# spotify-research/llark

Measured on AMD Instinct MI355X. Metric: clips/sec (25 s audio + 128-tok prompt) end-to-end fwd, higher is better.
Workload: dtype fp16x2-split(fp32-class) prior + bf16x2-split(fp32-class) llm; 1 GPU; configs[1]+llm: 8x25s clips -> Jukebox VQ-VAE+36-layer prior -> 240x4800 -> projector -> Llama-2-7B fwd (S=371) logits; clips_per_gpu=8, global_batch=8, audio_samples=1048576, seq_len=371, prior_depth=36, prior_precision=f16x2, prior_layernorm_folded=True, parallelism=dp1 (clip-sharded, no collective), debug_overrides=False

## Files before the change

include/llark_hip.h:

```cpp
#ifndef LLARK_HIP_H
#define LLARK_HIP_H

#include <stdint.h>

#ifdef __cplusplus
extern "C" {
#endif

typedef void* llark_stream_t;

enum {
    LLARK_OK = 0,
    LLARK_ERR_INVALID = -1,
    LLARK_ERR_UNSUPPORTED = -2,
    LLARK_ERR_LAUNCH = -3
};

enum { LLARK_F16 = 0, LLARK_BF16 = 1 };

enum {
    LLARK_EPI_F32 = 0,
    LLARK_EPI_RESID = 1,
    LLARK_EPI_QGELU_SPLIT = 2,
    LLARK_EPI_OUT16 = 3,
    LLARK_EPI_SWIGLU16 = 4,
    LLARK_EPI_SPLIT16 = 5,
    LLARK_EPI_SWIGLU_SPLIT = 6,
    LLARK_EPI_QGELU_SPLIT8 = 7
};

typedef struct llark_workspace* llark_workspace_t;
llark_workspace_t llark_workspace_create(void);
int llark_workspace_destroy(llark_workspace_t ws);

int llark_version(void);
const char* llark_last_error(void);
int llark_device_info(int device, char* arch_name, int arch_name_len);

int llark_resample_sinc_host(const float* x, int64_t n_in, double ratio, const double* win, const double* dwin, int nwin,
                             int num_table, float* y, int64_t n_out);

int llark_flac_info_host(const uint8_t* data, int64_t n, int* sample_rate, int* channels, int* bits_per_sample, int64_t* total_samples);
int llark_flac_decode_host(const uint8_t* data, int64_t n, int32_t* out, int64_t cap_frames, int64_t* decoded_frames, int verify_md5);

int llark_pack_conv_weight(const float* w, float* wp, int cout, int cin, int k, llark_stream_t stream);
int llark_conv1d_f32(const float* x, int n, int cin, int tin, const float* wp, const float* bias, int cout, int k,
                     int stride, int pad, int dil, float* y, int tout, llark_stream_t stream);
int llark_resblock_f32(const float* x, int n, int c, int t, const float* w1p, const float* b1, const float* w2p,
                       const float* b2, int dil, float* y, llark_stream_t stream);
int llark_codebook_norms_f32(const float* k, int bins, int emb, float* kk, llark_stream_t stream);
int llark_codebook_argmin(const float* x, int n, int emb, int t, const float* k, const float* kk, int bins,
                          int64_t* codes, float* min_dist, llark_stream_t stream);
void* llark_vqvae_plan_create(void);
void llark_vqvae_plan_destroy(void* plan);
int llark_vqvae_plan_add_conv(void* plan, const float* wp, const float* bias, int cin, int cout, int k, int stride, int pad);
int llark_vqvae_plan_add_resblock(void* plan, const float* w1p, const float* b1, const float* w2p, const float* b2, int width, int dil);
int llark_vqvae_encode(void* plan, const float* audio, int n, int t, float* buf0, float* buf1, long long buf_elems,
                       const float* codebook, const float* kk, int bins, int64_t* codes, int* t_out, llark_stream_t stream);
int llark_vqvae_stage_f16x2(const float* audio, const void* in_hi, const void* in_lo, int n, int cin, int tin, const float* w0_f32,
                            const void* w0_hi, const void* w0_lo, const float* b0, const void* wr_hi, const void* wr_lo,
                            const float* br, int depth, const int* dil, const void* wo_hi, const void* wo_lo, const float* bo,
                            const int* wexp, void* out_hi, void* out_lo, float* out_f32, llark_stream_t stream);
int llark_vqvae_pack_frag16(const float* w, int cout, int cin, int k, int perm1x1, int exp2, void* hi, void* lo, llark_stream_t stream);

int llark_codebook_argmin_tie(const float* x, int n, int emb, int t, const float* k, const float* kk, int bins, int64_t* codes,
                              float tie_a, float tie_b, int* flag_count, int* flag_list, int cap, llark_stream_t stream);
int llark_vqvae_fix_near_ties(void* plan, const float* audio, int n, int t_samples, int raw_to_tokens, const int* flag_list, int count,
                              int halo_tokens, int win_tokens, float* win, int* col, float* buf0, float* buf1, long long buf_elems,
                              const float* codebook, const float* kk, int bins, int64_t* codes, llark_stream_t stream);

int llark_prior_embed(const int64_t* z, int n, int t, int width, int bins, const float* x_emb, const float* pos_emb,
                      const float* x_cond, const float* y_cond, float* h, llark_stream_t stream);
int llark_layernorm_split_f16(const float* x, int ldx, int rows, int width, const float* gamma, const float* beta,
                              float eps, void* out_hi, void* out_lo, int ldo, llark_stream_t stream);
int llark_prior_attn(const float* qkv, int ldq, int n, int t, int n_state, int heads, int blocks, int pattern,
                     void* out_hi, void* out_lo, int ldo, llark_stream_t stream);
int llark_layernorm_split_lo8(const float* x, int ldx, int rows, int width, const float* gamma, const float* beta,
                              float eps, void* out_hi, int ldo, void* out_lo8, int ldo8, int sa, llark_stream_t stream);
int llark_prior_attn_lo8(const float* qkv, int ldq, int n, int t, int n_state, int heads, int blocks, int pattern,
                         void* out_hi, int ldo, void* out_lo8, int ldo8, int sa, llark_stream_t stream);
int llark_pool_window(const float* h, int n, int t, int width, int frame_len, float* out, int frames,
                      llark_stream_t stream);
int llark_pool_mean(const float* h, int n, int t, int width, const int* lens, float* out, llark_stream_t stream);
int llark_zero_pad16(void* plane, int rows, int ld, int from, llark_stream_t stream);

int llark_gemm16(int dtype, int split, int epilogue, const void* a_hi, const void* a_lo, int lda, const void* wt,
                 int ldw, const float* bias, int m, int n, int kp, float* c, int ldc, const float* resid, int ldr,
                 void* out_hi, void* out_lo, int ldo, llark_stream_t stream);
int llark_gemm16_ex(int variant, int dtype, int split, int epilogue, const void* a_hi, const void* a_lo, int lda,
                    const void* wt, int ldw, const float* bias, int m, int n, int kp, float* c, int ldc, const float* resid,
                    int ldr, void* out_hi, void* out_lo, int ldo, llark_stream_t stream);
int llark_gemm16_ws(int variant, int dtype, int split, int epilogue, const void* a_hi, const void* a_lo, int lda,
                    const void* wt, int ldw, const float* bias, int m, int n, int kp, float* c, int ldc, const float* resid,
                    int ldr, void* out_hi, void* out_lo, int ldo, llark_workspace_t ws, llark_stream_t stream);

int llark_gemm16_ln_takes(int m, int n, int kp);
int llark_gemm16_ln(int dtype, int epilogue, const void* a_hi, const void* a_lo, int lda, const void* wt, int ldw, const float* bias, int m,
                    int n, int kp, float* c, int ldc, const float* resid, int ldr, void* out_hi, void* out_lo, int ldo,
                    const float* ln_stat, const float* ln_vec, float* ln_part, llark_workspace_t ws, llark_stream_t stream);
int llark_ln_stats_finalize(const float* part, int rows, int nparts, int width, float eps, float* stat, llark_stream_t stream);
int llark_gemm16_ln_p(int dtype, int epilogue, const void* a_hi, const void* a_lo, int lda, const void* wt, int ldw, const float* bias, int m,
                      int n, int kp, float* c, int ldc, const float* resid, int ldr, void* out_hi, void* out_lo, int ldo,
                      const float* ln_stat, const float* ln_vec, float* ln_part, const float* ln_pred, llark_workspace_t ws, llark_stream_t stream);
int llark_ln_stats_finalize_p(const float* part, int rows, int nparts, int width, float eps, float* stat, float* pred, llark_stream_t stream);
int llark_gemm16_lnp_fragw(int dtype, const void* a_hi, const void* a_lo, int lda, const void* wfrag, const float* bias, int m, int n, int kp,
                           float* c, int ldc, const float* resid, int ldr, void* out_hi, void* out_lo, int ldo, const float* ln_vec,
                           float* ln_part, const float* ln_pred, llark_stream_t stream);
int llark_ln_row_pred(const float* x, int ldx, int rows, int width, float eps, float* pred, llark_stream_t stream);
int llark_gemm16_lo8(int epilogue, const void* a_hi, const void* a_lo8, int lda, int lda8, const void* wt, int ldw,
                     const void* w8, int ldw8, const float* bias, int m, int n, int kp, int sa, int sw, float* c, int ldc, const float* resid, int ldr,
                     void* out_hi, void* out_lo8, int ldo, int ldo8, llark_workspace_t ws, llark_stream_t stream);
int llark_pack_weight_lo8(const void* wt, int ldw, int n, int kp, int sw, void* out, int ldo, llark_stream_t stream);
int llark_pack_weight16_frag(const void* wt, int ldw, int n, int kp, void* dst, llark_stream_t stream);
int llark_gemm16_fragw(int variant, int dtype, int split, int epilogue, const void* a_hi, const void* a_lo, int lda,
                       const void* wfrag, const float* bias, int m, int n, int kp, float* c, int ldc, const float* resid,
                       int ldr, void* out_hi, void* out_lo, int ldo, llark_stream_t stream);
int llark_gemm16_fragw_whole_tiles(int split, int epilogue, int m, int n, int kp);
int llark_gemm16_fragw_rope_qkv(const void* a_hi, const void* a_lo, int lda, const void* wfrag, int kp, int batch, int s, int nh, int hd,
                                int pos0, const float* cos_t, const float* sin_t, int max_pos, void* q, void* k_cache, void* vt_cache,
                                void* q_lo, void* k_cache_lo, void* vt_cache_lo, int smax, llark_stream_t stream);
long long llark_gemm16_sk_scratch_bytes(void);
int llark_gemm16_fragw_sk(int variant, int dtype, int split, int epilogue, const void* a_hi, const void* a_lo, int lda,
                          const void* wfrag, const float* bias, int m, int n, int kp, float* c, int ldc, const float* resid,
                          int ldr, void* out_hi, void* out_lo, int ldo, void* scratch, long long scratch_bytes,
                          llark_stream_t stream);
int llark_gemm16_resid_rmsnorm(int dtype, int split, const void* a_hi, const void* a_lo, int lda, const void* wt, int ldw,
                               int m, int n, int kp, float* h, int ldh, const float* norm_w, float eps, void* x_hi,
                               void* x_lo, int ldx, llark_stream_t stream);
int llark_gemm16_rmsnorm_a(int dtype, int split, int epilogue, const float* x, int ldx, const float* norm_w, float eps,
                           const void* wt, int ldw, const float* bias, int m, int n, int kp, float* c, int ldc, void* out_hi,
                           void* out_lo, int ldo, llark_stream_t stream);
int llark_gemm16_batched(int dtype, int split, int epilogue, const void* a_hi, const void* a_lo, int lda, long long stride_a,
                         const void* wt, int ldw, long long stride_w, int m, int n, int kp, float* c, int ldc,
                         long long stride_c, void* out_hi, void* out_lo, int ldo, long long stride_o, int batch,
                         llark_stream_t stream);
int llark_pack_weight16(const void* w, int src_dtype, int transpose, int k, int n, void* wt, int dst_dtype, int ldw,
                        llark_stream_t stream);
int llark_split16(int dtype, const float* x, int ldx, int rows, int width, void* out_hi, void* out_lo, int ldo,
                  llark_stream_t stream);


int llark_embed_gather(const int64_t* ids, int rows, const void* table, int table_dtype, int vocab, int width,
                       float* out, int ldo, llark_stream_t stream);
int llark_rmsnorm_bf16(const float* x, int ldx, int rows, int width, const float* w, float eps, void* out_hi,
                       void* out_lo, int ldo, llark_stream_t stream);
int llark_rope_split_heads(const float* qkv, int batch, int s, int nh, int hd, int pos0, const float* cos_t,
                           const float* sin_t, int max_pos, void* q, void* k_cache, void* vt_cache, void* q_lo,
                           void* k_cache_lo, void* vt_cache_lo, int smax, llark_stream_t stream);
int llark_attn_prefill_bf16(const void* q, const void* k_cache, const void* vt_cache, const void* q_lo,
                            const void* k_cache_lo, const void* vt_cache_lo, int batch, int s, int nh, int hd, int past,
                            int smax, void* out, void* out_lo, llark_stream_t stream);
int llark_attn_decode_bf16(const void* q, const void* k_cache, const void* vt_cache, const void* q_lo,
                           const void* k_cache_lo, const void* vt_cache_lo, int batch, int nh, int hd, int total, int smax,
                           void* out, void* out_lo, llark_stream_t stream);
int llark_attn_prefill_bf16_alibi(const void* q, const void* k_cache, const void* vt_cache, const void* q_lo,
                                  const void* k_cache_lo, const void* vt_cache_lo, int batch, int s, int nh, int hd, int past,
                                  int smax, void* out, void* out_lo, const float* alibi_slopes, llark_stream_t stream);
int llark_attn_decode_bf16_alibi(const void* q, const void* k_cache, const void* vt_cache, const void* q_lo,
                                 const void* k_cache_lo, const void* vt_cache_lo, int batch, int nh, int hd, int total, int smax,
                                 void* out, void* out_lo, const float* alibi_slopes, llark_stream_t stream);

int llark_gemv16_dma(int split, int epilogue, const void* a_hi, const void* a_lo, int lda, const void* wt, int ldw, const float* bias,
                     int m, int n, int kp, float* c, int ldc, const float* resid, int ldr, void* out_hi, void* out_lo, int ldo,
                     llark_stream_t stream);
int llark_gemv16_dma_rmsnorm(int split, int epilogue, const float* x, int ldx, const float* norm_w, float eps, const void* wt, int ldw,
                             const float* bias, int m, int n, int kp, float* c, int ldc, void* out_hi, void* out_lo, int ldo,
                             llark_stream_t stream);

int llark_gemm16_t(int dtype, int epilogue, int trans_a, int trans_b, const void* a, int lda, const void* wt, int ldw, int m, int n,
                   int kp, float* c, int ldc, const float* resid, int ldr, llark_stream_t stream);
int llark_gemm16_t_sumsq(int dtype, int epilogue, int trans_a, int trans_b, const void* a, int lda, const void* wt, int ldw, int m, int n,
                         int kp, float* c, int ldc, const float* resid, int ldr, double* sumsq, llark_stream_t stream);

int llark_gemm16_t_ex(int variant, int dtype, int epilogue, int trans_a, int trans_b, const void* a, int lda, const void* wt, int ldw, int m,
                      int n, int kp, float* c, int ldc, const float* resid, int ldr, double* sumsq, llark_stream_t stream);

int llark_attn_prefill_bf16_lse(const void* q, const void* k_cache, const void* vt_cache, int batch, int s, int nh, int hd,
                                int smax, void* out, float* lse, const float* alibi_slopes, llark_stream_t stream);
int llark_attn_backward_bf16(const void* q, const void* k_cache, const void* v_rm, const void* dO, const void* o, const float* lse,
                             float* dsum, int batch, int s, int nh, int hd, int smax, float* dq, float* dk, float* dv,
                             const float* alibi_slopes, llark_stream_t stream);

int llark_layernorm_bf16(const float* x, int ldx, int rows, int width, const float* gamma, const float* beta, float eps,
                         void* out_hi, void* out_lo, int ldo, llark_stream_t stream);
int llark_layernorm_f32(const float* x, int ldx, int rows, int width, const float* gamma, const float* beta, float eps,
                        float* y, int ldy, llark_stream_t stream);
int llark_clamp_f32(float* x, long long n, float limit, llark_stream_t stream);
int llark_clamp_bwd_bf16(const float* x, long long n, float limit, void* dy, llark_stream_t stream);
int llark_scale_f32(float* x, long long n, float a, llark_stream_t stream);
int llark_gelu_split_bf16(const float* x, int ldx, int rows, int width, void* out_hi, void* out_lo, int ldo,
                          llark_stream_t stream);
int llark_layernorm_bwd(const float* x, int ldx, const float* gamma, const float* dy, int ldy, int rows, int width, float eps,
                        float* dx, int lddx, float* dgamma, float* dbeta, int accumulate, llark_stream_t stream);
int llark_gelu_bwd(const float* up, const float* dact, long long n, float* dup32, void* dup16, llark_stream_t stream);
int llark_causal_softmax_rows_alibi(const float* scores, int batch, int s, float scale, const float* slopes, int nh, void* p_out,
                                    int ldp, llark_stream_t stream);
int llark_clap_logmel(const float* wav, int batch, int n, int quantize_int16, const float* window, const float* twiddle,
                      const float* melw, const int* mel_lo, const int* mel_hi, float* out, llark_stream_t stream);
int llark_clap_patchify(const float* x, int batch, int frames, int mel, const float* bn_mean, const float* bn_scale,
                        const float* bn_bias, const int* tap_idx, const float* tap_w, int spec, int patch, void* out_hi,
                        void* out_lo, int ldo, llark_stream_t stream);
int llark_clap_window_attn(const float* qkv, int ldq, int batch, int H, int W, int C, int heads, int window, int shift,
                           const float* bias_table, void* out_hi, void* out_lo, void* out_hi_dup, int ldo, llark_stream_t stream);
int llark_layernorm_bf16_dup(const float* x, int ldx, int rows, int width, const float* gamma, const float* beta, float eps,
                             void* out_hi, void* out_lo, void* out_hi_dup, int ldo, llark_stream_t stream);
int llark_gemm16_act(int variant, int dtype, int split, int epilogue, const void* a_hi, const void* a_lo, int lda, const void* wt,
                     int ldw, const float* bias, int m, int n, int kp, void* out_hi, void* out_lo, void* out_hi_dup, int ldo,
                     int act, llark_stream_t stream);
int llark_clap_patch_merge(const float* x, int ldx, int batch, int H, int W, int C, float* out, int ldo, llark_stream_t stream);
int llark_mean_rows_f32(const float* x, int ldx, int batch, int L, int C, float* out, int ldo, llark_stream_t stream);
int llark_relu_split_bf16(const float* x, int ldx, int rows, int width, void* out_hi, void* out_lo, int ldo, llark_stream_t stream);
int llark_l2_normalize_rows(float* x, int ldx, int rows, int width, float eps, llark_stream_t stream);

int llark_attn_decode_rope_bf16(const float* qkv, int batch, int nh, int hd, int pos, const int* pos_dev, const float* cos_t,
                                const float* sin_t, int max_pos, void* k_cache, void* vt_cache, void* k_cache_lo, void* vt_cache_lo,
                                int smax, void* out, void* out_lo, const float* alibi_slopes, llark_stream_t stream);
#define LLARK_ROW_IDLE 0
#define LLARK_ROW_ACTIVE 1
#define LLARK_ROW_FINISHED 2
int llark_attn_decode_rope_bf16_rows(const float* qkv, int batch, int nh, int hd, const int* pos_rows, const float* cos_t,
                                     const float* sin_t, int max_pos, void* k_cache, void* vt_cache, void* k_cache_lo, void* vt_cache_lo,
                                     int smax, void* out, void* out_lo, const float* alibi_slopes, llark_stream_t stream);
int llark_decode_advance_rows(const float* logits, int ldl, int vocab, int batch, const int64_t* choice, int* pos_rows, int* state,
                              int64_t* next_ids, int64_t* out_col, int ld_out, int64_t eos, int64_t pad, llark_stream_t stream);
int llark_rope_split_heads_dpos(const float* qkv, int batch, int nh, int hd, const int* pos_dev, const float* cos_t,
                                const float* sin_t, void* q, void* k_cache, void* vt_cache, void* q_lo, void* k_cache_lo,
                                void* vt_cache_lo, int smax, llark_stream_t stream);
int llark_attn_decode_bf16_dpos(const void* q, const void* k_cache, const void* vt_cache, const void* q_lo,
                                const void* k_cache_lo, const void* vt_cache_lo, int batch, int nh, int hd,
// ... 62 lines not shown
```

llark_amd/_lib.py:

```python
from __future__ import annotations

import ctypes
import os
import subprocess
from ctypes import c_char_p, c_double, c_float, c_int, c_int64, c_uint, c_void_p

_HERE = os.path.dirname(os.path.abspath(__file__))
LIB_PATH = os.environ.get("LLARK_HIP_LIB") or os.path.join(_HERE, "libllark_hip.so")
CSRC = os.path.join(_HERE, "csrc")

_lib = None


class LlarkHipError(RuntimeError):
    pass


def build(force: bool = False, verbose: bool = False) -> str:
    srcs = [os.path.join(CSRC, f) for f in os.listdir(CSRC) if f.endswith((".hip", ".h"))]
    srcs.append(os.path.join(_HERE, "..", "include", "llark_hip.h"))
    stale = (not os.path.exists(LIB_PATH)) or any(
        os.path.getmtime(s) > os.path.getmtime(LIB_PATH) for s in srcs if os.path.exists(s)
    )
    if force or stale:
        cmd = ["make", "-C", CSRC, "-j8"] + (["-B"] if force else [])
        res = subprocess.run(cmd, capture_output=not verbose, text=True)
        if res.returncode != 0:
            raise LlarkHipError(f"building libllark_hip.so failed:\n{res.stdout}\n{res.stderr}")
    return LIB_PATH


_P = c_void_p
_SIGS = {
    "llark_version": [],
    "llark_device_info": [c_int, c_char_p, c_int],
    "llark_resample_sinc_host": [_P, c_int64, c_double, _P, _P, c_int, c_int, _P, c_int64],
    "llark_flac_info_host": [_P, c_int64, _P, _P, _P, _P],
    "llark_flac_decode_host": [_P, c_int64, _P, c_int64, _P, c_int],
    "llark_pack_conv_weight": [_P, _P, c_int, c_int, c_int, _P],
    "llark_conv1d_f32": [_P, c_int, c_int, c_int, _P, _P, c_int, c_int, c_int, c_int, c_int, _P, c_int, _P],
    "llark_resblock_f32": [_P, c_int, c_int, c_int, _P, _P, _P, _P, c_int, _P, _P],
    "llark_codebook_norms_f32": [_P, c_int, c_int, _P, _P],
    "llark_codebook_argmin": [_P, c_int, c_int, c_int, _P, _P, c_int, _P, _P, _P],
    "llark_prior_embed": [_P, c_int, c_int, c_int, c_int, _P, _P, _P, _P, _P, _P],
    "llark_layernorm_split_f16": [_P, c_int, c_int, c_int, _P, _P, c_float, _P, _P, c_int, _P],
    "llark_prior_attn": [_P, c_int, c_int, c_int, c_int, c_int, c_int, c_int, _P, _P, c_int, _P],
    "llark_pool_window": [_P, c_int, c_int, c_int, c_int, _P, c_int, _P],
    "llark_pool_mean": [_P, c_int, c_int, c_int, _P, _P, _P],
    "llark_zero_pad16": [_P, c_int, c_int, c_int, _P],
    "llark_vqvae_plan_add_conv": [_P, _P, _P, c_int, c_int, c_int, c_int, c_int],
    "llark_vqvae_plan_add_resblock": [_P, _P, _P, _P, _P, c_int, c_int],
    "llark_vqvae_encode": [_P, _P, c_int, c_int, _P, _P, c_int64, _P, _P, c_int, _P, _P, _P],
    "llark_codebook_argmin_tie": [_P, c_int, c_int, c_int, _P, _P, c_int, _P, c_float, c_float, _P, _P, c_int, _P],
    "llark_vqvae_fix_near_ties": [_P, _P, c_int, c_int, c_int, _P, c_int, c_int, c_int, _P, _P, _P, _P, c_int64, _P, _P, c_int, _P, _P],
    "llark_vqvae_stage_f16x2": [_P, _P, _P, c_int, c_int, c_int, _P, _P, _P, _P, _P, _P, _P, c_int, _P, _P, _P, _P, _P, _P, _P, _P, _P],
    "llark_vqvae_pack_frag16": [_P, c_int, c_int, c_int, c_int, c_int, _P, _P, _P],
    "llark_gemm16": [c_int, c_int, c_int, _P, _P, c_int, _P, c_int, _P, c_int, c_int, c_int, _P, c_int, _P, c_int,
                     _P, _P, c_int, _P],
    "llark_gemm16_ex": [c_int, c_int, c_int, c_int, _P, _P, c_int, _P, c_int, _P, c_int, c_int, c_int, _P, c_int, _P, c_int,
                        _P, _P, c_int, _P],
    "llark_gemm16_ws": [c_int, c_int, c_int, c_int, _P, _P, c_int, _P, c_int, _P, c_int, c_int, c_int, _P, c_int, _P, c_int,
                        _P, _P, c_int, _P, _P],
    "llark_gemm16_lo8": [c_int, _P, _P, c_int, c_int, _P, c_int, _P, c_int, _P, c_int, c_int, c_int, c_int, c_int, _P, c_int, _P, c_int,
                         _P, _P, c_int, c_int, _P, _P],
    "llark_pack_weight_lo8": [_P, c_int, c_int, c_int, c_int, _P, c_int, _P],
    "llark_gemm16_ln_takes": [c_int, c_int, c_int],
    "llark_gemm16_ln": [c_int, c_int, _P, _P, c_int, _P, c_int, _P, c_int, c_int, c_int, _P, c_int, _P, c_int, _P, _P, c_int, _P, _P, _P, _P, _P],
    "llark_ln_stats_finalize": [_P, c_int, c_int, c_int, c_float, _P, _P],
    "llark_gemm16_fragw_whole_tiles": [c_int, c_int, c_int, c_int, c_int],
    "llark_gemm16_ln_p": [c_int, c_int, _P, _P, c_int, _P, c_int, _P, c_int, c_int, c_int, _P, c_int, _P, c_int, _P, _P, c_int, _P, _P, _P, _P, _P, _P],
    "llark_gemm16_lnp_fragw": [c_int, _P, _P, c_int, _P, _P, c_int, c_int, c_int, _P, c_int, _P, c_int, _P, _P, c_int, _P, _P, _P, _P],
    "llark_ln_stats_finalize_p": [_P, c_int, c_int, c_int, c_float, _P, _P, _P],
    "llark_ln_row_pred": [_P, c_int, c_int, c_int, c_float, _P, _P],
    "llark_workspace_destroy": [_P],
    "llark_layernorm_split_lo8": [_P, c_int, c_int, c_int, _P, _P, c_float, _P, c_int, _P, c_int, c_int, _P],
    "llark_prior_attn_lo8": [_P, c_int, c_int, c_int, c_int, c_int, c_int, c_int, _P, c_int, _P, c_int, c_int, _P],
    "llark_pack_weight16_frag": [_P, c_int, c_int, c_int, _P, _P],
    "llark_gemm16_fragw": [c_int, c_int, c_int, c_int, _P, _P, c_int, _P, _P, c_int, c_int, c_int, _P, c_int, _P, c_int,
                           _P, _P, c_int, _P],
    "llark_gemm16_fragw_sk": [c_int, c_int, c_int, c_int, _P, _P, c_int, _P, _P, c_int, c_int, c_int, _P, c_int, _P, c_int,
                              _P, _P, c_int, _P, c_int64, _P],
    "llark_gemm16_fragw_rope_qkv": [_P, _P, c_int, _P, c_int, c_int, c_int, c_int, c_int, c_int, _P, _P, c_int, _P, _P, _P, _P, _P, _P, c_int, _P],
    "llark_gemm16_resid_rmsnorm": [c_int, c_int, _P, _P, c_int, _P, c_int, c_int, c_int, c_int, _P, c_int, _P, c_float, _P, _P,
                                   c_int, _P],
    "llark_gemm16_rmsnorm_a": [c_int, c_int, c_int, _P, c_int, _P, c_float, _P, c_int, _P, c_int, c_int, c_int, _P, c_int, _P, _P,
                               c_int, _P],
    "llark_gemm16_batched": [c_int, c_int, c_int, _P, _P, c_int, c_int64, _P, c_int, c_int64, c_int, c_int, c_int, _P, c_int,
                             c_int64, _P, _P, c_int, c_int64, c_int, _P],
    "llark_pack_weight16": [_P, c_int, c_int, c_int, c_int, _P, c_int, c_int, _P],
    "llark_split16": [c_int, _P, c_int, c_int, c_int, _P, _P, c_int, _P],
    "llark_embed_gather": [_P, c_int, _P, c_int, c_int, c_int, _P, c_int, _P],
    "llark_rmsnorm_bf16": [_P, c_int, c_int, c_int, _P, c_float, _P, _P, c_int, _P],
    "llark_attn_prefill_bf16_alibi": [_P, _P, _P, _P, _P, _P, c_int, c_int, c_int, c_int, c_int, c_int, _P, _P, _P, _P],
    "llark_attn_decode_bf16_alibi": [_P, _P, _P, _P, _P, _P, c_int, c_int, c_int, c_int, c_int, _P, _P, _P, _P],
    "llark_gemv16_dma": [c_int, c_int, _P, _P, c_int, _P, c_int, _P, c_int, c_int, c_int, _P, c_int, _P, c_int, _P, _P, c_int, _P],
    "llark_gemv16_dma_rmsnorm": [c_int, c_int, _P, c_int, _P, c_float, _P, c_int, _P, c_int, c_int, c_int, _P, c_int, _P, _P, c_int, _P],
    "llark_gemm16_t": [c_int, c_int, c_int, c_int, _P, c_int, _P, c_int, c_int, c_int, c_int, _P, c_int, _P, c_int, _P],
    "llark_gemm16_t_ex": [c_int, c_int, c_int, c_int, c_int, _P, c_int, _P, c_int, c_int, c_int, c_int, _P, c_int, _P, c_int, _P, _P],
    "llark_gemm16_t_sumsq": [c_int, c_int, c_int, c_int, _P, c_int, _P, c_int, c_int, c_int, c_int, _P, c_int, _P, c_int, _P, _P],
    "llark_attn_prefill_bf16_lse": [_P, _P, _P, c_int, c_int, c_int, c_int, c_int, _P, _P, _P, _P],
    "llark_attn_backward_bf16": [_P, _P, _P, _P, _P, _P, _P, c_int, c_int, c_int, c_int, c_int, _P, _P, _P, _P, _P],
    "llark_layernorm_bf16": [_P, c_int, c_int, c_int, _P, _P, c_float, _P, _P, c_int, _P],
    "llark_layernorm_f32": [_P, c_int, c_int, c_int, _P, _P, c_float, _P, c_int, _P],
    "llark_clamp_f32": [_P, c_int64, c_float, _P],
    "llark_clamp_bwd_bf16": [_P, c_int64, c_float, _P, _P],
    "llark_sumsq_f32": [_P, c_int64, _P, c_int, _P],
    "llark_scale_f32": [_P, c_int64, c_float, _P],
    "llark_gelu_split_bf16": [_P, c_int, c_int, c_int, _P, _P, c_int, _P],
    "llark_layernorm_bwd": [_P, c_int, _P, _P, c_int, c_int, c_int, c_float, _P, c_int, _P, _P, c_int, _P],
    "llark_gelu_bwd": [_P, _P, c_int64, _P, _P, _P],
    "llark_causal_softmax_rows_alibi": [_P, c_int, c_int, c_float, _P, c_int, _P, c_int, _P],
    "llark_clap_logmel": [_P, c_int, c_int, c_int, _P, _P, _P, _P, _P, _P, _P],
    "llark_clap_patchify": [_P, c_int, c_int, c_int, _P, _P, _P, _P, _P, c_int, c_int, _P, _P, c_int, _P],
    "llark_clap_window_attn": [_P, c_int, c_int, c_int, c_int, c_int, c_int, c_int, c_int, _P, _P, _P, _P, c_int, _P],
    "llark_layernorm_bf16_dup": [_P, c_int, c_int, c_int, _P, _P, c_float, _P, _P, _P, c_int, _P],
    "llark_gemm16_act": [c_int, c_int, c_int, c_int, _P, _P, c_int, _P, c_int, _P, c_int, c_int, c_int, _P, _P, _P, c_int, c_int, _P],
    "llark_clap_patch_merge": [_P, c_int, c_int, c_int, c_int, c_int, _P, c_int, _P],
    "llark_mean_rows_f32": [_P, c_int, c_int, c_int, c_int, _P, c_int, _P],
    "llark_relu_split_bf16": [_P, c_int, c_int, c_int, _P, _P, c_int, _P],
    "llark_l2_normalize_rows": [_P, c_int, c_int, c_int, c_float, _P],
    "llark_attn_decode_rope_bf16": [_P, c_int, c_int, c_int, c_int, _P, _P, _P, c_int, _P, _P, _P, _P, c_int, _P, _P, _P, _P],
    "llark_attn_decode_rope_bf16_rows": [_P, c_int, c_int, c_int, _P, _P, _P, c_int, _P, _P, _P, _P, c_int, _P, _P, _P, _P],
    "llark_decode_advance_rows": [_P, c_int, c_int, c_int, _P, _P, _P, _P, _P, c_int, c_int64, c_int64, _P],
    "llark_rope_split_heads_dpos": [_P, c_int, c_int, c_int, _P, _P, _P, _P, _P, _P, _P, _P, _P, c_int, _P],
    "llark_attn_decode_bf16_dpos": [_P, _P, _P, _P, _P, _P, c_int, c_int, c_int, _P, c_int, _P, _P, _P],
    "llark_rope_split_heads": [_P, c_int, c_int, c_int, c_int, c_int, _P, _P, c_int, _P, _P, _P, _P, _P, _P, c_int, _P],
    "llark_attn_prefill_bf16": [_P, _P, _P, _P, _P, _P, c_int, c_int, c_int, c_int, c_int, c_int, _P, _P, _P],
    "llark_attn_decode_bf16": [_P, _P, _P, _P, _P, _P, c_int, c_int, c_int, c_int, c_int, _P, _P, _P],
    "llark_cross_entropy_shifted": [_P, c_int, c_int, c_int, c_int, _P, c_int64, _P, _P, _P],
    "llark_transpose16": [_P, c_int, c_int, c_int, _P, c_int, c_int, c_int64, c_int64, _P],
    "llark_split_heads16": [_P, c_int, c_int, c_int, c_int, _P, _P],
    "llark_causal_softmax_rows": [_P, c_int, c_int, c_float, _P, c_int, _P],
    "llark_attn_ds": [_P, _P, c_int, c_int, c_float, _P, c_int, _P],
    "llark_rope_merge_bwd": [_P, _P, _P, _P, _P, c_int, c_int, c_int, c_int, c_int, _P, _P],
    "llark_rmsnorm_bwd": [_P, _P, _P, c_int, c_int, c_float, _P, c_int, _P, _P],
    "llark_rmsnorm_bwd_out16": [_P, _P, _P, c_int, c_int, c_float, _P, c_int, _P, _P, c_int, _P],
    "llark_swiglu_fwd": [_P, c_int, c_int, _P, _P],
    "llark_swiglu_bwd": [_P, _P, c_int, c_int, _P, _P],
    "llark_cross_entropy_bwd": [_P, c_int, c_int, c_int, c_int, _P, _P, _P, c_float, _P, c_int, _P],
    "llark_colsum_f32": [_P, c_int, c_int, c_int, _P, _P],
    "llark_gather_rows_f32": [_P, c_int, _P, c_int, c_int, _P, c_int, _P],
    "llark_scatter_add_rows_f32": [_P, c_int, _P, c_int, c_int, _P, c_int, _P],
    "llark_adamw": [c_int, _P, _P, _P, _P, c_int64, c_float, c_float, c_float, c_float, c_float, c_int, c_float, _P],
    "llark_adamw_clip": [c_int, _P, _P, _P, _P, c_int64, c_float, c_float, c_float, c_float, c_float, c_int, c_float, _P, c_float, _P],
    "llark_gemm16_fragw_swiglu_train": [c_int, _P, c_int, _P, c_int, c_int, c_int, _P, c_int, _P, c_int, _P],
    "llark_pack_frag_t16": [_P, c_int, c_int, c_int, _P, _P],
    "llark_gemm16_ta_fragw": [c_int, _P, c_int, _P, c_int, c_int, c_int, _P, c_int, _P, c_int, _P, _P],
    "llark_pack_frag_t16x16": [_P, c_int, c_int, c_int, _P, _P],
    "llark_gemm16_ta_fragw16": [c_int, _P, c_int, _P, c_int, c_int, c_int, _P, c_int, _P, c_int, _P, _P],
    "llark_gemm16_fragw_rope_qkv_train": [_P, c_int, _P, c_int, c_int, c_int, c_int, c_int, c_int, _P, _P, c_int, _P, _P, _P, c_int, _P, _P],
    "llark_attn_backward_bf16_fused": [_P, _P, _P, _P, c_int, _P, _P, _P, c_int, c_int, c_int, c_int, c_int, _P, _P, c_int, c_int, _P, _P],
    "llark_gemv16_dma_blocks": [c_int, c_int],
    "llark_gemv16_dma_chain": [c_int, c_int, _P, _P, c_int, _P, c_int, _P, c_float, _P, c_int, _P, c_int, c_int, c_int, _P, c_int, _P, c_int, _P, _P, c_int, _P, c_uint, _P, _P],
    "llark_attn_decode_rope_bf16_chain": [_P, c_int, c_int, c_int, c_int, _P, _P, _P, c_int, _P, _P, _P, _P, c_int, _P, _P, _P, _P, _P],
    "llark_adamw_twins": [_P, _P, _P, _P, c_int, c_int, c_float, c_float, c_float, c_float, c_float, c_int, c_float, _P, c_float, _P, c_int, _P, _P],
}


def declared_symbols():
    return sorted(list(_SIGS.keys()) + ["llark_last_error", "llark_vqvae_plan_create", "llark_vqvae_plan_destroy", "llark_workspace_create", "llark_gemm16_sk_scratch_bytes"])


_recorder = None
current_label = None


class _RecordingProxy:
    def __init__(self, real, rec):
        self._real, self._rec = real, rec

    def __getattr__(self, name):
        fn = getattr(self._real, name)
        if not name.startswith("llark_") or name == "llark_last_error":
            return fn
        rec = self._rec

        def call(*args):
            rc = fn(*args)
            rec.append((fn, name, args, current_label))
            return rc

        return call


def set_recorder(rec) -> None:
    global _recorder
    _recorder = rec


def lib():
    L = _real_lib()
    return _RecordingProxy(L, _recorder) if _recorder is not None else L


def _real_lib():
    global _lib
    if _lib is None:
        if not os.path.exists(LIB_PATH):
            build()
# ... 27 lines not shown
```

llark_amd/csrc/gemm.hip:

```cpp

#ifndef GEMM_ABLATE
#define GEMM_ABLATE 0
#endif

#include <new>

#include "gemm_core.h"
#include "gemm_rope_epi.h"
#include "gemm_bd.h"
#include "gemm_bda_loop.h"

namespace llark {

template <typename T, bool SPLIT, int EPI, typename C>
__device__ __forceinline__ void gemm_tile(const GemmParams& p, int bid, char* smem) {
    typedef typename Mfma<T>::frag frag;
    constexpr int STAGE = (SPLIT ? 2 : 1) * C::A_BYTES + C::B_BYTES;
    constexpr int OFF_L = C::A_BYTES, OFF_W = (SPLIT ? 2 : 1) * C::A_BYTES;
    constexpr int NS = C::NSTAGE;

    const int lane = threadIdx.x & 63;
    const int w = __builtin_amdgcn_readfirstlane(threadIdx.x >> 6);
    const int wm = w / C::WN, wn = w % C::WN;

// ... 647 lines not shown
        case 1: return dispatch<T, Cfg1>(p, split, epi, s);
        case 2: return dispatch<T, Cfg2>(p, split, epi, s);
        case 11: return dispatch<T, Cfg11>(p, split, epi, s);
        case 12: return dispatch<T, Cfg12>(p, split, epi, s);
        case 13:
            if (split) break;
            switch (epi) {
                case EPI_F32: return launch_gemm<T, false, EPI_F32, Cfg13>(p, s);
                case EPI_RESID: return launch_gemm<T, false, EPI_RESID, Cfg13>(p, s);
                case EPI_OUT16: return launch_gemm<T, false, EPI_OUT16, Cfg13>(p, s);
                case EPI_SWIGLU16: return launch_gemm<T, false, EPI_SWIGLU16, Cfg13>(p, s);
            }
            break;
        case 32: {
            if (split && ws && ws->cus % 8 == 0) {
                GemmParams q = p;
                const int dt = std::is_same<T, half_t>::value ? LLARK_F16 : LLARK_BF16;
                if (ws_begin(ws, q, s) == 0) {
                    const int rc = launch_gemm256x(q, dt, epi, s, ws->cus);
                    if (rc != -1000) {
                        ws_end(ws, cdiv(p.M, 256) * cdiv(p.N, 256), ws->cus / 8);
                        return rc;
                    }
                }
            }
        }
        [[fallthrough]];
        case 31: {
            if (split && ws && ws->cus % 8 == 0) {
                GemmParams q = p;
                const int dt = std::is_same<T, half_t>::value ? LLARK_F16 : LLARK_BF16;
                if (ws_begin(ws, q, s) == 0) {
                    const int rc = launch_gemm256n(q, dt, epi, s, ws->cus);
                    if (rc != -1000) {
                        ws_end(ws, cdiv(p.M, 256) * cdiv(p.N, 256), ws->cus / 8);
                        return rc;
                    }
                }
            }
        }
        [[fallthrough]];
        case 30: {
            if (split && ws && ws->cus % 8 == 0) {
                GemmParams q = p;
                const int dt = std::is_same<T, half_t>::value ? LLARK_F16 : LLARK_BF16;
                if (ws_begin(ws, q, s) == 0) {
                    const int rc = launch_gemm256(q, dt, epi, s, ws->cus);
                    if (rc != -1000) {
                        ws_end(ws, cdiv(p.M, 256) * cdiv(p.N, 256), ws->cus / 8);
                        return rc;
                    }
                }
            }
        }
        [[fallthrough]];
        case 20: {
            const int rc = dispatch_persist<T, Cfg12>(p, split, epi, s, ws);
            return rc == -1000 ? dispatch<T, Cfg12>(p, split, epi, s) : rc;
        }
    }
    set_error("gemm: unknown tile variant %d", variant);
    return LLARK_ERR_INVALID;
}

}

using namespace llark;

static int pick_variant(int split, int m, int n, int kp, bool has_ws) {
    if (m <= 128) return 0;
    if (!split && kp % 64 == 0 && n < 16384) return 11;
    if (n < 256) return 0;
    if (kp % 64 != 0) return kp < 2048 ? 1 : 2;
    const bool persist = has_ws;
    if (split && persist && kp >= 128 && (long)cdiv(m, 256) * cdiv(n, 256) >= 384) return kp >= 2048 ? 32 : 31;
    if (kp < 2048) return 12;
    if (m >= 16384 && persist) return 20;
    if (!split && n < 16384) return 11;
    return 12;
}

static int gemm16_impl(int variant, int dtype, int split, int epilogue, const void* a_hi, const void* a_lo, int lda,
                       const void* wt, int ldw, const float* bias, int m, int n, int kp, float* c, int ldc,
                       const float* resid, int ldr, void* out_hi, void* out_lo, int ldo, int batch, long long sa,
                       long long sw, long long sc, long long sr, long long so, llark_stream_t stream, void* out_hi2 = nullptr,
                       int act = 0, llark_workspace* ws = nullptr) {
    LLARK_REQUIRE(a_hi && wt && m > 0 && n > 0 && kp > 0, "gemm16: null pointer or empty problem");
    LLARK_REQUIRE(kp % 64 == 0 || (kp % 32 == 0 && variant < 10),
                  "gemm16: kp=%d must be a multiple of the K-step (zero-pad K)", kp);
    LLARK_REQUIRE(lda % 8 == 0 && ldw % 8 == 0 && lda >= kp && ldw >= kp, "gemm16: lda/ldw must be >= kp and multiples of 8");
    LLARK_REQUIRE(!split || a_lo, "gemm16: split mode needs the lo plane");
    LLARK_REQUIRE(((uintptr_t)a_hi & 15) == 0 && ((uintptr_t)wt & 15) == 0 && (!a_lo || ((uintptr_t)a_lo & 15) == 0),
                  "gemm16: operands must be 16-byte aligned");
    if (epilogue == EPI_F32 || epilogue == EPI_RESID) LLARK_REQUIRE(c && ldc >= n, "gemm16: fp32 output missing");
    if (epilogue == EPI_RESID) LLARK_REQUIRE(resid && ldr >= n, "gemm16: residual missing");
    if (epilogue == EPI_QGELU_SPLIT || epilogue == EPI_SPLIT16) LLARK_REQUIRE(out_hi && out_lo && ldo >= n, "gemm16: split outputs missing");
    if (epilogue == EPI_OUT16) LLARK_REQUIRE(out_hi && ldo >= n, "gemm16: 16-bit output missing");
    if (IS_SWIGLU(epilogue)) LLARK_REQUIRE(out_hi && n % 64 == 0 && ldo >= n / 2, "gemm16: swiglu needs n%%64==0 and an output");
    if (epilogue == EPI_SWIGLU_SPLIT) LLARK_REQUIRE(out_lo, "gemm16: swiglu-split needs the lo output");
    GemmParams p = {};
    p.Ahi = a_hi; p.Alo = a_lo; p.lda = lda; p.Wt = wt; p.ldw = ldw; p.bias = bias;
    p.M = m; p.N = n; p.Kp = kp; p.C = c; p.ldc = ldc; p.R = resid; p.ldr = ldr;
    p.Ohi = out_hi; p.Olo = out_lo; p.ldo = ldo; p.Ohi2 = out_hi2; p.act = act;
    p.tiles_m = p.tiles_n = 0;
    p.batch = batch; p.sA = sa; p.sW = sw; p.sC = sc; p.sR = sr; p.sO = so;
    hipStream_t s = (hipStream_t)stream;
    if (variant < 0 && m <= 16 && batch <= 1 && act == 0 && !out_hi2) {
        int rc = 1;
        if (dtype == LLARK_F16) rc = dispatch_skinny<half_t>(p, split != 0, epilogue, s);
        else if (dtype == LLARK_BF16) rc = dispatch_skinny<bf16_t>(p, split != 0, epilogue, s);
        if (rc != 1) return rc;
    }
    if (variant < 0) variant = pick_variant(split, m, n, kp, ws != nullptr);
    if (dtype == LLARK_F16) return dispatch_variant<half_t>(variant, p, split != 0, epilogue, s, ws);
    if (dtype == LLARK_BF16) return dispatch_variant<bf16_t>(variant, p, split != 0, epilogue, s, ws);
    set_error("gemm16: unknown dtype %d", dtype);
    return LLARK_ERR_INVALID;
}

extern "C" int llark_gemm16_ex(int variant, int dtype, int split, int epilogue, const void* a_hi, const void* a_lo, int lda,
                               const void* wt, int ldw, const float* bias, int m, int n, int kp, float* c, int ldc,
                               const float* resid, int ldr, void* out_hi, void* out_lo, int ldo,
                               llark_stream_t stream) {
    return gemm16_impl(variant, dtype, split, epilogue, a_hi, a_lo, lda, wt, ldw, bias, m, n, kp, c, ldc, resid, ldr, out_hi,
                       out_lo, ldo, 0, 0, 0, 0, 0, 0, stream);
}

extern "C" int llark_gemm16_ws(int variant, int dtype, int split, int epilogue, const void* a_hi, const void* a_lo, int lda,
                               const void* wt, int ldw, const float* bias, int m, int n, int kp, float* c, int ldc,
                               const float* resid, int ldr, void* out_hi, void* out_lo, int ldo, llark_workspace_t ws,
                               llark_stream_t stream) {
    return gemm16_impl(variant, dtype, split, epilogue, a_hi, a_lo, lda, wt, ldw, bias, m, n, kp, c, ldc, resid, ldr, out_hi,
                       out_lo, ldo, 0, 0, 0, 0, 0, 0, stream, nullptr, 0, ws);
}

extern "C" int llark_gemm16_ln_takes(int m, int n, int kp) { return gemm256x_takes(m, n, kp) ? 1 : 0; }

extern "C" int llark_gemm16_ln(int dtype, int epilogue, const void* a_hi, const void* a_lo, int lda, const void* wt, int ldw, const float* bias, int m,
                               int n, int kp, float* c, int ldc, const float* resid, int ldr, void* out_hi, void* out_lo, int ldo,
                               const float* ln_stat, const float* ln_vec, float* ln_part, llark_workspace_t ws, llark_stream_t stream) {
    return llark_gemm16_ln_p(dtype, epilogue, a_hi, a_lo, lda, wt, ldw, bias, m, n, kp, c, ldc, resid, ldr, out_hi, out_lo, ldo, ln_stat, ln_vec, ln_part,
                             nullptr, ws, stream);
}

extern "C" int llark_gemm16_ln_p(int dtype, int epilogue, const void* a_hi, const void* a_lo, int lda, const void* wt, int ldw, const float* bias, int m,
                                 int n, int kp, float* c, int ldc, const float* resid, int ldr, void* out_hi, void* out_lo, int ldo,
                                 const float* ln_stat, const float* ln_vec, float* ln_part, const float* ln_pred, llark_workspace_t ws,
                                 llark_stream_t stream) {
    LLARK_REQUIRE(a_hi && a_lo && wt && ln_vec && ws && m > 0 && n > 0 && kp > 0, "gemm16_ln: null pointer or empty problem");
    LLARK_REQUIRE(ln_pred == nullptr || ln_part != nullptr, "gemm16_ln: ln_pred belongs to the producer role (ln_part)");
    LLARK_REQUIRE((ln_stat != nullptr) != (ln_part != nullptr), "gemm16_ln: exactly one of ln_stat (consumer) / ln_part (producer) must be given");
    LLARK_REQUIRE(lda % 8 == 0 && ldw % 8 == 0 && lda >= kp && ldw >= kp, "gemm16_ln: lda/ldw must be >= kp and multiples of 8");
    if (ln_part) LLARK_REQUIRE(epilogue == EPI_RESID && c && resid && out_hi && out_lo && ldc >= n && ldr >= n && ldo >= n, "gemm16_ln: the producer role is LLARK_EPI_RESID with c, resid and the operand planes");
    else LLARK_REQUIRE((epilogue == EPI_F32 && c && ldc >= n) || (epilogue == EPI_QGELU_SPLIT && out_hi && out_lo && ldo >= n), "gemm16_ln: the consumer role is LLARK_EPI_F32 or LLARK_EPI_QGELU_SPLIT");
    if (!gemm256x_takes(m, n, kp) || ws->cus % 8) {
        set_error("gemm16_ln: m=%d n=%d kp=%d is not a shape the 256x256 tile takes", m, n, kp);
        return LLARK_ERR_UNSUPPORTED;
    }
    GemmParams p = {};
    p.Ahi = a_hi; p.Alo = a_lo; p.lda = lda; p.Wt = wt; p.ldw = ldw; p.bias = bias;
    p.M = m; p.N = n; p.Kp = kp; p.C = c; p.ldc = ldc; p.R = resid; p.ldr = ldr;
    p.Ohi = out_hi; p.Olo = out_lo; p.ldo = ldo;
    p.ln_stat = ln_stat; p.ln_vec = ln_vec; p.ln_part = ln_part; p.ln_pred = ln_pred;
    hipStream_t s = (hipStream_t)stream;
    if (ws_begin(ws, p, s)) {
        set_error("gemm16_ln: workspace without counters");
        return LLARK_ERR_INVALID;
    }
    const int rc = launch_gemm256x(p, dtype, epilogue, s, ws->cus);
    if (rc == -1000) {
        set_error("gemm16_ln: operands do not meet the tile's alignment rules");
        return LLARK_ERR_UNSUPPORTED;
    }
    ws_end(ws, cdiv(m, 256) * cdiv(n, 256), ws->cus / 8);
    return rc;
}

extern "C" int llark_gemm16_lnp_fragw(int dtype, const void* a_hi, const void* a_lo, int lda, const void* wfrag, const float* bias, int m, int n, int kp,
                                      float* c, int ldc, const float* resid, int ldr, void* out_hi, void* out_lo, int ldo, const float* ln_vec,
                                      float* ln_part, const float* ln_pred, llark_stream_t stream) {
    LLARK_REQUIRE(a_hi && a_lo && wfrag && ln_vec && ln_part && c && resid && out_hi && out_lo && m > 0 && n > 0 && kp > 0,
                  "gemm16_lnp_fragw: null pointer or empty problem");
    LLARK_REQUIRE(kp % 64 == 0 && lda % 8 == 0 && lda >= kp && ldc >= n && ldr >= n && ldo >= n, "gemm16_lnp_fragw: kp must be a multiple of 64, lda >= kp a multiple of 8, ldc / ldr / ldo >= n");
    LLARK_REQUIRE(((uintptr_t)a_hi & 15) == 0 && ((uintptr_t)a_lo & 15) == 0 && ((uintptr_t)wfrag & 15) == 0, "gemm16_lnp_fragw: operands must be 16-byte aligned");
    GemmParams p = {};
    p.Ahi = a_hi; p.Alo = a_lo; p.lda = lda; p.Wt = wfrag; p.ldw = 0; p.bias = bias; p.M = m; p.N = n; p.Kp = kp;
    p.C = c; p.ldc = ldc; p.R = resid; p.ldr = ldr; p.Ohi = out_hi; p.Olo = out_lo; p.ldo = ldo;
    p.ln_vec = ln_vec; p.ln_part = ln_part; p.ln_pred = ln_pred;
    const int rc = launch_gemm_bda_lnp(p, dtype, (hipStream_t)stream);
    if (rc == -1000) {
        set_error("gemm16_lnp_fragw: needs f16 / bf16 planes, kp >= 192, n %% 4 == 0, 16-byte aligned fp32 rows (ldc, ldr multiples of 4) and 8-byte aligned plane rows (ldo a multiple of 4)");
        return LLARK_ERR_UNSUPPORTED;
    }
    return rc;
}

extern "C" llark_workspace_t llark_workspace_create(void) {
    int dev = 0, cus = 0;
    if (hipGetDevice(&dev) != hipSuccess || hipDeviceGetAttribute(&cus, hipDeviceAttributeMultiprocessorCount, dev) != hipSuccess) {
        set_error("workspace_create: cannot query the current device");
        return nullptr;
    }
    llark_workspace* ws = new (std::nothrow) llark_workspace();
    if (!ws) { set_error("workspace_create: out of host memory"); return nullptr; }
    ws->device = dev; ws->cus = cus; ws->base = 0; ws->counters = nullptr;
#ifdef G256X_PROF
    if (const char* e = getenv("LLARK_G256X_CUS")) ws->cus = atoi(e);
#endif
    if (hipMalloc((void**)&ws->counters, LLARK_WS_BYTES) != hipSuccess || hipMemset(ws->counters, 0, LLARK_WS_BYTES) != hipSuccess) {
        set_error("workspace_create: cannot allocate %d bytes of device memory", LLARK_WS_BYTES);
        if (ws->counters) (void)hipFree(ws->counters);
        delete ws;
        return nullptr;
    }
    return ws;
}

extern "C" int llark_workspace_destroy(llark_workspace_t ws) {
    if (!ws) return LLARK_OK;
    if (ws->counters) (void)hipFree(ws->counters);
    delete ws;
    return LLARK_OK;
}

extern "C" int llark_gemm16_lo8(int epilogue, const void* a_hi, const void* a_lo8, int lda, int lda8, const void* wt, int ldw,
                                const void* w8, int ldw8, const float* bias, int m, int n, int kp, int sa, int sw, float* c, int ldc, const float* resid,
                                int ldr, void* out_hi, void* out_lo8, int ldo, int ldo8, llark_workspace_t ws,
                                llark_stream_t stream) {
    LLARK_REQUIRE(a_hi && a_lo8 && wt && w8 && ws && m > 0 && n > 0, "gemm16_lo8: null pointer (a_hi / a_lo8 / wt / w8 / ws) or empty problem");
    LLARK_REQUIRE(kp % 64 == 0 && kp >= 128, "gemm16_lo8: kp=%d must be a multiple of 64 and >= 128 (zero-pad K)", kp);
    LLARK_REQUIRE(lda % 8 == 0 && ldw % 8 == 0 && lda >= kp && ldw >= kp && lda8 >= kp && lda8 % 16 == 0,
                  "gemm16_lo8: lda/ldw/lda8 must be >= kp, lda/ldw multiples of 8, lda8 a multiple of 16");
    LLARK_REQUIRE(((uintptr_t)a_hi & 15) == 0 && ((uintptr_t)wt & 15) == 0 && ((uintptr_t)a_lo8 & 15) == 0,
                  "gemm16_lo8: operands must be 16-byte aligned");
    LLARK_REQUIRE(sa >= 0 && sa <= 40 && sw >= -40 && sw <= 40, "gemm16_lo8: scale exponents out of range (sa=%d sw=%d)", sa, sw);
    LLARK_REQUIRE(ldw8 >= kp && ldw8 % 16 == 0 && ((uintptr_t)w8 & 15) == 0, "gemm16_lo8: w8 plane needs ldw8 >= kp, ldw8 %% 16 == 0 and 16-byte alignment");
    if (epilogue == EPI_F32 || epilogue == EPI_RESID) LLARK_REQUIRE(c && ldc >= n, "gemm16_lo8: fp32 output missing");
    if (epilogue == EPI_RESID) LLARK_REQUIRE(resid && ldr >= n, "gemm16_lo8: residual missing");
    if (epilogue == EPI_QGELU_SPLIT8)
        LLARK_REQUIRE(out_hi && out_lo8 && ldo >= n && ldo8 >= ((n + 63) & ~63) && ldo8 % 64 == 0,
                      "gemm16_lo8: split outputs missing (ldo8 must cover n rounded up to 64 and be a multiple of 64)");
    LLARK_REQUIRE(epilogue == EPI_F32 || epilogue == EPI_RESID || epilogue == EPI_QGELU_SPLIT8, "gemm16_lo8: unsupported epilogue %d", epilogue);
    LLARK_REQUIRE(ws->cus > 0 && ws->cus % 8 == 0, "gemm16_lo8: device with %d CUs is not supported (needs a multiple of 8)", ws->cus);
    GemmParams p = {};
    p.Ahi = a_hi; p.Alo = a_lo8; p.lda = lda; p.lda8 = lda8; p.Wt = wt; p.ldw = ldw; p.bias = bias;
    p.M = m; p.N = n; p.Kp = kp; p.C = c; p.ldc = ldc; p.R = resid; p.ldr = ldr;
    p.Ohi = out_hi; p.Olo = out_lo8; p.ldo = ldo; p.ldo8 = ldo8; p.lo8_sa = sa; p.lo8_sw = sw; p.W8 = w8; p.ldw8 = ldw8;
    hipStream_t s = (hipStream_t)stream;
    if (ws_begin(ws, p, s)) { set_error("gemm16_lo8: workspace unusable"); return LLARK_ERR_LAUNCH; }
    const int rc = launch_gemm256_lo8n(p, epilogue, s, ws->cus);
    if (rc == -1000) { set_error("gemm16_lo8: problem outside the kernel's range (32-bit operand offsets)"); return LLARK_ERR_UNSUPPORTED; }
    ws_end(ws, cdiv(m, 256) * cdiv(n, 256), ws->cus / 8);
    return rc;
}

extern "C" int llark_gemm16_act(int variant, int dtype, int split, int epilogue, const void* a_hi, const void* a_lo, int lda,
                                const void* wt, int ldw, const float* bias, int m, int n, int kp, void* out_hi, void* out_lo,
                                void* out_hi_dup, int ldo, int act, llark_stream_t stream) {
    LLARK_REQUIRE(epilogue == EPI_SPLIT16 || epilogue == EPI_OUT16, "gemm16_act: epilogue must be SPLIT16 or OUT16");
    LLARK_REQUIRE(act == 0 || act == 2, "gemm16_act: act must be 0 (none) or 2 (exact GELU)");
    LLARK_REQUIRE(!out_hi_dup || epilogue == EPI_SPLIT16, "gemm16_act: the duplicate hi plane belongs to the SPLIT16 epilogue");
    return gemm16_impl(variant, dtype, split, epilogue, a_hi, a_lo, lda, wt, ldw, bias, m, n, kp, nullptr, 0, nullptr, 0, out_hi,
                       out_lo, ldo, 0, 0, 0, 0, 0, 0, stream, out_hi_dup, act);
}

extern "C" int llark_pack_weight16_frag(const void* wt, int ldw, int n, int kp, void* dst, llark_stream_t stream) {
    LLARK_REQUIRE(wt && dst && n > 0 && kp > 0 && kp % 64 == 0 && ldw >= kp && ldw % 8 == 0, "pack_weight16_frag: bad arguments (kp must be a multiple of 64)");
    LLARK_REQUIRE(((uintptr_t)wt & 15) == 0 && ((uintptr_t)dst & 15) == 0, "pack_weight16_frag: pointers must be 16-byte aligned");
    const long long total = (long long)cdiv(n, 32) * (kp / 16) * 64;
    pack_frag_kernel<<<dim3((unsigned)((total + 255) / 256)), 256, 0, (hipStream_t)stream>>>((const unsigned short*)wt, ldw, n, kp, (uint4*)dst, total);
    return check_launch("pack_weight16_frag");
}

static int llark_device_cus() {
    static int cached[64] = {0};
    int dev = 0;
    if (hipGetDevice(&dev) != hipSuccess || dev < 0 || dev >= 64) return 256;
    if (!cached[dev]) {
        int cus = 0;
        if (hipDeviceGetAttribute(&cus, hipDeviceAttributeMultiprocessorCount, dev) != hipSuccess || cus <= 0) return 256;
        cached[dev] = cus;
    }
    return cached[dev];
}

static bool fragw_sk_rule(bool split, int m, int n, int kp) {
    const long long tiles_bd0 = (long long)cdiv(m, CfgBD0::BM) * cdiv(n, CfgBD0::BN);
    return (split && tiles_bd0 < 2LL * llark_device_cus()) ||
           (!split && (4 * tiles_bd0 <= 2LL * llark_device_cus() || (tiles_bd0 < 2LL * llark_device_cus() && kp >= 8192)));
}
static bool fragw_small_tiles(int dtype, bool split, int epilogue, int n) {
    if (GEMM_BDA >= 2 && dtype == LLARK_BF16) return false;
    return !split && !IS_SWIGLU(epilogue) && n <= 4096;
}

extern "C" int llark_gemm16_fragw_whole_tiles(int split, int epilogue, int m, int n, int kp) {
    if (m <= 0 || n <= 0 || kp <= 0) return 0;
    return (!fragw_sk_rule(split != 0, m, n, kp) && !fragw_small_tiles(LLARK_BF16, split != 0, epilogue, n)) ? 1 : 0;
}

static int gemm16_fragw_impl(int variant, int dtype, int split, int epilogue, const void* a_hi, const void* a_lo, int lda,
                             const void* wfrag, const float* bias, int m, int n, int kp, float* c, int ldc,
                             const float* resid, int ldr, void* out_hi, void* out_lo, int ldo, void* scratch, long long scratch_bytes,
                             llark_stream_t stream) {
    LLARK_REQUIRE(a_hi && wfrag && m > 0 && n > 0 && kp > 0 && kp % 64 == 0, "gemm16_fragw: null pointer / empty problem / kp not a multiple of 64");
    LLARK_REQUIRE(lda % 8 == 0 && lda >= kp, "gemm16_fragw: lda must be >= kp and a multiple of 8");
    LLARK_REQUIRE(!split || a_lo, "gemm16_fragw: split mode needs the lo plane");
// ... 167 lines not shown
```

llark_amd/csrc/gemm256x.hip:

```cpp
#include "gemm_core.h"

namespace llark {

struct Cfg256X {
    static constexpr int BK = 64, BM = 256, BN = 256, NW = 8, THREADS = 512, MINW = 2;
    static constexpr int TM = 4, TN = 8;
    static constexpr int ROWB = 128, UNIT = 128 * ROWB;
    static constexpr int NW_SLOTS = 3, NA_SLOTS = 7;
    static constexpr int O_W = 0, O_A = NW_SLOTS * UNIT;
    static constexpr int LDS = O_A + NA_SLOTS * UNIT;
    static_assert(LDS == 160 * 1024, "LDS map");
};

template <typename T>
struct Mfma16;
template <>
struct Mfma16<half_t> {
    typedef half8_t frag;
    typedef half4_t out4;
    static __device__ __forceinline__ f32x4_t run(frag a, frag b, f32x4_t c) { return __builtin_amdgcn_mfma_f32_16x16x32_f16(a, b, c, 0, 0, 0); }
};
template <>
struct Mfma16<bf16_t> {
    typedef bf16x8_t frag;
// ... 373 lines not shown
                                if constexpr (i >= r0 + 10 && i < r0 + 14) al[i - r0 - 10][1] = *(const frag*)(smem + vAs[1] + 8192 + (i - r0 - 10) * 2048);
                                if constexpr (i == 16) bf[0] = *(const frag*)(smem + vWs[1]);
                                if constexpr (i == 17) bf[1] = *(const frag*)(smem + vWs[1] + 2048);
                                if constexpr (i >= 18 && i < 22) dmaop(std::integral_constant<int, i - 18>{});
                            } else {
                                if constexpr (i == r0) bf[2] = *(const frag*)(smem + vWs[0] + 2 * 2048);
                                if constexpr (i == r0 + 1) bf[3] = *(const frag*)(smem + vWs[0] + 3 * 2048);
                                if constexpr (i >= r0 + 2 && i < r0 + 6) dmaop(std::integral_constant<int, i - r0 - 2>{});
                                if constexpr (i == 16) bf[0] = *(const frag*)(smem + vWs[1]);
                                if constexpr (i == 17) bf[1] = *(const frag*)(smem + vWs[1] + 2048);
                            }
                        } else {
                            if constexpr (i == 2) bf[2] = *(const frag*)(smem + vWs[1] + 2 * 2048);
                            if constexpr (i == 3) bf[3] = *(const frag*)(smem + vWs[1] + 3 * 2048);
                            if constexpr (i >= 4 && i < 6) midop(std::integral_constant<int, i - 4>{});
                        }
                        __builtin_amdgcn_sched_barrier(0);
                    });
                });
            };

            auto kstep = [&](auto right_tag, int k, int aq, int wL) __attribute__((always_inline)) {
                const int kn = k + 1 < nk ? k + 1 : nk - 1;
                const int wR = wL + 1 >= 3 ? wL - 2 : wL + 1, wN = wL + 2 >= 3 ? wL - 1 : wL + 2;
                const int an = wrap7(aq + 4);
                const int amine = wrap7(aq + wm) * C::UNIT;
                auto reqQ = [&](int j, int lo_plane, int slot) __attribute__((always_inline)) {
                    const unsigned vo = j == 0 ? voA[0] : j == 1 ? voA[1] : j == 2 ? voA[2] : voA[3];
                    dma(lo_plane ? rAl : rAh, vo, kn << 7, C::O_A + slot * C::UNIT + wb + (lo_plane ? 8192 : 0));
                };
                auto reqW = [&](int right, int piece, int slot) __attribute__((always_inline)) {
                    dma(rW, voW[2 * right + piece], kn << 7, C::O_W + slot * C::UNIT + piece * 8192 + wb);
                };
                phase(std::integral_constant<int, 0>{}, std::integral_constant<int, 4>{}, std::true_type{}, amine, wL * C::UNIT,
                      [&](auto ic) __attribute__((always_inline)) { constexpr int i = decltype(ic)::value; reqQ(i >> 1, i & 1, wrap7(an + (i >> 1))); },
                      [&](auto ic) __attribute__((always_inline)) { reqW(0, decltype(ic)::value, wN); });
                __builtin_amdgcn_s_barrier();
                phase(std::integral_constant<int, 1>{}, std::integral_constant<int, 4>{}, right_tag, amine, wR * C::UNIT,
                      [&](auto ic) __attribute__((always_inline)) { constexpr int i = decltype(ic)::value; reqQ(2 + (i >> 1), i & 1, wrap7(an + 2 + (i >> 1))); },
                      [&](auto ic) __attribute__((always_inline)) { reqW(1, decltype(ic)::value, wL); });
                VMCNT(2);
                __builtin_amdgcn_s_barrier();
            };

#if G256X_PRIO
            if (w >= 4) __builtin_amdgcn_s_setprio(1);
#endif
            if (w >= 4) __builtin_amdgcn_s_barrier();
            {
                int aq = 0, wL = 0;
                if (n0 + 128 < p.N) {
                    for (int k = 0; k < nk; ++k) {
                        kstep(std::true_type{}, k, aq, wL);
                        aq = wrap7(aq + 4);
                        wL = wL + 2 >= 3 ? wL - 1 : wL + 2;
                    }
                } else {
                    for (int k = 0; k < nk; ++k) {
                        kstep(std::false_type{}, k, aq, wL);
                        aq = wrap7(aq + 4);
                        wL = wL + 2 >= 3 ? wL - 1 : wL + 2;
                    }
                }
            }
            if (w < 4) __builtin_amdgcn_s_barrier();
            VMCNT(0);
            __builtin_amdgcn_s_barrier();
            PROF_STAMP(1);
            f32x4_t bias[C::TN], res0[C::TN], res1[C::TN];
            f32x4_t gv;
            float2 st[C::TM];
            if (LN != 0) gv = gamma_load(p, n0, wn, lane);
            else epilogue_load_bias(p, bias, n0, wn, lane);
            if (LN == 1 || LN == 2) {
                const bool whole = m0 + C::BM <= p.M;
                const float* rowst = LN == 1 ? p.ln_stat : p.ln_pred;
#pragma unroll
                for (int tm = 0; tm < C::TM; ++tm) {
                    const int m = m0 + wm * 64 + tm * 16 + (lane & 15);
                    st[tm] = (rowst != nullptr && (whole || m < p.M)) ? *(const float2*)(rowst + 2 * (size_t)m) : make_float2(0.f, 1.f);
                }
            }
            epilogue_load_resid<EPI>(p, res0, 0, m0, n0, wm, wn, lane);
            epilogue_load_resid<EPI>(p, res1, 1, m0, n0, wm, wn, lane);
            if (LN != 0) gamma_park(smem, gv, w, lane);
            __builtin_amdgcn_sched_barrier(0);
            if (ch + 1 < nchunks) {
                if (threadIdx.x == 0) __hip_atomic_fetch_add(cnt, 1, __ATOMIC_RELAXED, __HIP_MEMORY_SCOPE_AGENT);
                arrived = true;
                const int nl = (ch + 1) * p.slots + slot_id;
                primed = nl < bandn;
                if (primed) {
                    int m1, n1;
                    tile_of(band0 + nl, m1, n1);
                    set_offsets(m1, n1);
                    prologue();
                }
            }
            __builtin_amdgcn_sched_barrier(0);
            epilogue_store<T, EPI, LN>(p, smem, acc, res0, bias, st, 0, m0, n0, wm, wn, lane);
            __builtin_amdgcn_sched_barrier(0);
            epilogue_load_resid<EPI>(p, res0, 2, m0, n0, wm, wn, lane);
            __builtin_amdgcn_sched_barrier(0);
            epilogue_store<T, EPI, LN>(p, smem, acc, res1, bias, st, 1, m0, n0, wm, wn, lane);
            __builtin_amdgcn_sched_barrier(0);
            epilogue_load_resid<EPI>(p, res1, 3, m0, n0, wm, wn, lane);
            __builtin_amdgcn_sched_barrier(0);
            epilogue_store<T, EPI, LN>(p, smem, acc, res0, bias, st, 2, m0, n0, wm, wn, lane);
            epilogue_store<T, EPI, LN>(p, smem, acc, res1, bias, st, 3, m0, n0, wm, wn, lane);
            PROF_STAMP(2);
            ++prof_tile;
        }
        if (ch + 1 < nchunks) {
            if (threadIdx.x == 0) {
                if (!arrived) __hip_atomic_fetch_add(cnt, 1, __ATOMIC_RELAXED, __HIP_MEMORY_SCOPE_AGENT);
                const int target = p.sync_base + (ch + 1 - G256X_RUNAHEAD) * p.slots;
                for (int it = 0; it < 100000 && __hip_atomic_load(cnt, __ATOMIC_RELAXED, __HIP_MEMORY_SCOPE_AGENT) - target < 0; ++it)
                    __builtin_amdgcn_s_sleep(8);
            }
            __builtin_amdgcn_s_barrier();
        }
    }
#ifdef G256X_PROF
    VMCNT(0);
    __builtin_amdgcn_s_barrier();
    PROF_STAMP(0);
#endif
}

template <typename T, int EPI, int LN>
static int launch256x(GemmParams p, hipStream_t s, int cus) {
    typedef Cfg256X C;
    auto kern = gemm256x_kernel<T, EPI, LN>;
    static PerDeviceOnce once;
    if (once.first()) {
        if (hipFuncSetAttribute((const void*)kern, hipFuncAttributeMaxDynamicSharedMemorySize, C::LDS) != hipSuccess) return -1000;
    }
    p.tiles_m = cdiv(p.M, C::BM);
    p.tiles_n = cdiv(p.N, C::BN);
#ifdef G256X_PROF
    if (const char* e = getenv("LLARK_G256X_PROF_BUF")) p.prof = (long long*)strtoull(e, nullptr, 0);
#endif
    p.slots = cus / 8;
    kern<<<dim3(cus), C::THREADS, C::LDS, s>>>(p);
    return check_launch("gemm256x");
}

template <typename T>
static int dispatch256x(const GemmParams& p, int epi, hipStream_t s, int cus) {
    if (p.ln_stat) {
        if (!p.ln_vec || p.ln_part) return -1000;
        if (epi == EPI_F32) return launch256x<T, EPI_F32, 1>(p, s, cus);
        if (epi == EPI_QGELU_SPLIT) return launch256x<T, EPI_QGELU_SPLIT, 1>(p, s, cus);
        return -1000;
    }
    if (p.ln_part) {
        if (!p.ln_vec || epi != EPI_RESID || !p.Ohi || !p.Olo) return -1000;
        return launch256x<T, EPI_RESID, 2>(p, s, cus);
    }
    switch (epi) {
        case EPI_F32: return launch256x<T, EPI_F32, 0>(p, s, cus);
        case EPI_RESID: return launch256x<T, EPI_RESID, 0>(p, s, cus);
        case EPI_QGELU_SPLIT: return launch256x<T, EPI_QGELU_SPLIT, 0>(p, s, cus);
        case EPI_SPLIT16: if (p.act == 0 && p.Ohi2 == nullptr) return launch256x<T, EPI_SPLIT16, 0>(p, s, cus);
    }
    return -1000;
}

bool gemm256x_takes(int m, int n, int kp) {
    return kp % 64 == 0 && kp >= 128 && n % 4 == 0 && m > 0 && (long)cdiv(m, 256) * cdiv(n, 256) >= 384;
}

int launch_gemm256x(const GemmParams& p, int dtype, int epi, hipStream_t s, int cus) {
    if (!p.Alo || p.Kp % 64 != 0 || p.Kp < 128 || p.batch > 1 || !p.sync || cus <= 0 || cus % 8) return -1000;
    if ((long long)p.M * p.lda * 2 >= (1ll << 31) || (long long)p.N * p.ldw * 2 >= (1ll << 31)) return -1000;
    if (p.N % 4) return -1000;
    if (p.bias && ((uintptr_t)p.bias & 15)) return -1000;
    if ((epi == EPI_F32 || epi == EPI_RESID) && (p.ldc % 4 || ((uintptr_t)p.C & 15))) return -1000;
    if (epi == EPI_RESID && (p.ldr % 4 || ((uintptr_t)p.R & 15))) return -1000;
    if ((epi == EPI_QGELU_SPLIT || epi == EPI_SPLIT16 || p.ln_part) && (p.ldo % 4 || ((uintptr_t)p.Ohi & 7) || ((uintptr_t)p.Olo & 7))) return -1000;
    if ((p.ln_stat || p.ln_part) && (!p.ln_vec || ((uintptr_t)p.ln_vec & 15) || ((uintptr_t)p.ln_stat & 7) || ((uintptr_t)p.ln_part & 7) || ((uintptr_t)p.ln_pred & 7))) return -1000;
    if (dtype == LLARK_F16) return dispatch256x<half_t>(p, epi, s, cus);
    if (dtype == LLARK_BF16) return dispatch256x<bf16_t>(p, epi, s, cus);
    return -1000;
}

}
```

llark_amd/csrc/prior.hip:

```cpp
#include <type_traits>

#include "common.h"

namespace llark {

__global__ void prior_embed_kernel(const long long* __restrict__ z, const float4* __restrict__ x_emb,
                                   const float4* __restrict__ pos_emb, const float4* __restrict__ x_cond,
                                   const float4* __restrict__ y_cond, float4* __restrict__ h, int n, int t, int w4,
                                   int bins) {
    const size_t total = (size_t)n * t * w4;
    for (size_t i = (size_t)blockIdx.x * blockDim.x + threadIdx.x; i < total; i += (size_t)gridDim.x * blockDim.x) {
        const int c = (int)(i % w4);
        const size_t row = i / w4;
        const int tt = (int)(row % t);
        const size_t nn = row / t;
        float4 e;
        if (tt == 0) {
            e = y_cond[c];
        } else {
            long long code = z[nn * t + tt - 1];
            code = code < 0 ? 0 : (code >= bins ? bins - 1 : code);
            e = x_emb[(size_t)code * w4 + c];
        }
        const float4 pe = pos_emb[(size_t)tt * w4 + c];
// ... 588 lines not shown
                const int d = 32 * s + 8 * g + 2 * e;
                const bool in = d < hd;
                const float2 a = *(const float2*)(qrow + (in ? d : 0));
                const float x = in ? a.x : 0.0f, y = in ? a.y : 0.0f;
                const half_t hx = (half_t)x, hy = (half_t)y;
                qh[s][2 * e] = hx;
                qh[s][2 * e + 1] = hy;
                ql[s][2 * e] = (half_t)(x - (float)hx);
                ql[s][2 * e + 1] = (half_t)(y - (float)hy);
            }
        }
    }

    const int krow = 8 * (c >> 2) + (c & 3);
    const int kswz = a16::swz(krow);
    f32x4_t sc[2][4];
#pragma unroll
    for (int kt = 0; kt < 2; ++kt) {
        if (kt >= ntile) break;
        if (kt) __syncthreads();
        a16::store_rows16h<NK32>(R, tile, wv * 16, nkeys - kt * 64, hd, lane);
        __syncthreads();
        if (kt + 1 < ntile) load_rows16(R, wv * 16, kbase, rowbase + k0 + (size_t)(kt + 1) * 64 * ks, ks, p.ldq, nkeys - (kt + 1) * 64, hd, lane);
        else load_rows16(R, wv * 16, vbase, rowbase + k0, ks, p.ldq, nkeys, hd, lane);
        f32x4_t acc[4];
#pragma unroll
        for (int t = 0; t < 4; ++t) acc[t] = f32x4_t{0.f, 0.f, 0.f, 0.f};
#pragma unroll
        for (int s = 0; s < NK32; ++s) {
            half8_t kh[4], kl[4];
#pragma unroll
            for (int t = 0; t < 4; ++t) {
                const int o = (krow + 32 * (t >> 1) + 4 * (t & 1)) * a16::PITCH + (((4 * s + g) ^ kswz) << 4);
                kh[t] = *(const half8_t*)(tile + o);
                kl[t] = *(const half8_t*)(tile + a16::PLANE + o);
            }
#pragma unroll
            for (int t = 0; t < 4; ++t) acc[t] = a16::mfma(kh[t], qh[s], acc[t]);
#pragma unroll
            for (int t = 0; t < 4; ++t) acc[t] = a16::mfma(kh[t], ql[s], acc[t]);
#pragma unroll
            for (int t = 0; t < 4; ++t) acc[t] = a16::mfma(kl[t], qh[s], acc[t]);
        }
        const int i = wv * 16 + c;
#pragma unroll
        for (int t = 0; t < 4; ++t)
#pragma unroll
            for (int r = 0; r < 4; ++r) {
                const int j = kt * 64 + 32 * (t >> 1) + 8 * g + 4 * (t & 1) + r;
                const bool ok = (j < nkeys) && (!causal || (j <= i + coff));
                sc[kt][t][r] = ok ? acc[t][r] * p.scale2 : -INFINITY;
            }
    }

    {
        float mx = -INFINITY;
#pragma unroll
        for (int kt = 0; kt < 2; ++kt) {
            if (kt >= ntile) break;
#pragma unroll
            for (int t = 0; t < 4; ++t)
                mx = fmaxf(fmaxf(fmaxf(sc[kt][t][0], sc[kt][t][1]), fmaxf(sc[kt][t][2], sc[kt][t][3])), mx);
        }
        mx = fmaxf(mx, __shfl_xor(mx, 16));
        mx = fmaxf(mx, __shfl_xor(mx, 32));
        float sum = 0.0f;
#pragma unroll
        for (int kt = 0; kt < 2; ++kt) {
            if (kt >= ntile) break;
#pragma unroll
            for (int t = 0; t < 4; ++t)
#pragma unroll
                for (int r = 0; r < 4; ++r) {
                    const float ex = mx > -INFINITY ? expf(sc[kt][t][r] - mx) : 0.0f;
                    sc[kt][t][r] = ex;
                    sum += ex;
                }
        }
        sum += __shfl_xor(sum, 16);
        sum += __shfl_xor(sum, 32);
        const float inv = sum > 0.0f ? 1.0f / sum : 0.0f;
#pragma unroll
        for (int kt = 0; kt < 2; ++kt) {
            if (kt >= ntile) break;
#pragma unroll
            for (int t = 0; t < 4; ++t) sc[kt][t] *= inv;
        }
    }

    f32x4_t o[NDT];
#pragma unroll
    for (int dt = 0; dt < NDT; ++dt) o[dt] = f32x4_t{0.f, 0.f, 0.f, 0.f};
#pragma unroll
    for (int kt = 0; kt < 2; ++kt) {
        if (kt >= ntile) break;
        __syncthreads();
        a16::store_rows16h<NK32>(R, tile, wv * 16, nkeys - kt * 64, hd, lane);
        __syncthreads();
        if (kt + 1 < ntile) load_rows16(R, wv * 16, vbase, rowbase + k0 + (size_t)(kt + 1) * 64 * ks, ks, p.ldq, nkeys - (kt + 1) * 64, hd, lane);
#pragma unroll
        for (int u = 0; u < 2; ++u) {
            half8_t ph, pl;
#pragma unroll
            for (int e = 0; e < 8; ++e) {
                const float pv = sc[kt][2 * u + (e >> 2)][e & 3];
                const half_t h = (half_t)pv;
                ph[e] = h;
                pl[e] = (half_t)(pv - (float)h);
            }
#pragma unroll
            for (int dt = 0; dt < NDT; ++dt) {
                const half8_t vh = a16::tr_frag(tile, 32 * u, 16 * dt, g, c);
                const half8_t vl = a16::tr_frag(tile + a16::PLANE, 32 * u, 16 * dt, g, c);
                o[dt] = a16::mfma(vh, ph, o[dt]);
                o[dt] = a16::mfma(vh, pl, o[dt]);
                o[dt] = a16::mfma(vl, ph, o[dt]);
            }
        }
    }
    __syncthreads();
    float* sT = sm;
    {
        float* orow = sT + (wv * 16 + c) * ATT_KP + 4 * g;
#pragma unroll
        for (int dt = 0; dt < NDT; ++dt) *(f32x4_t*)(orow + dt * 16) = o[dt];
    }
    {
        typedef _Float16 half2_t __attribute__((ext_vector_type(2)));
        const int npair = hd >> 1;
        const float sm8 = __builtin_ldexpf(1.0f, p.sa);
        for (int idx = lane; idx < 16 * npair; idx += 64) {
            const int rr = idx / npair, pr = idx - rr * npair;
            const int i = wv * 16 + rr;
            if (i >= nq) break;
            const float2 x = *(const float2*)(sT + i * ATT_KP + 2 * pr);
            const size_t tok = rowbase + q0 + (size_t)i * qs;
            half2_t h;
            h[0] = (half_t)x.x;
            h[1] = (half_t)x.y;
            *(half2_t*)(p.ohi + tok * p.ldo + hcol + 2 * pr) = h;
            if (p.lo8) {
                const unsigned q8 = fp8_e4m3_sat((x.x - (float)h[0]) * sm8) | (fp8_e4m3_sat((x.y - (float)h[1]) * sm8) << 8);
                *(unsigned short*)((unsigned char*)p.olo + tok * p.ldo8 + lo8_pos(hcol + 2 * pr)) = (unsigned short)q8;
            } else {
                half2_t l;
                l[0] = (half_t)(x.x - (float)h[0]);
                l[1] = (half_t)(x.y - (float)h[1]);
                *(half2_t*)(p.olo + tok * p.ldo + hcol + 2 * pr) = l;
            }
        }
    }
}

__global__ void pool_window_kernel(const float* __restrict__ h, float* __restrict__ out, int t, int width,
                                   int frame_len, int frames) {
    const int f = blockIdx.x, n = blockIdx.y;
    const float* src = h + ((size_t)n * t + (size_t)f * frame_len) * width;
    float* dst = out + ((size_t)n * frames + f) * width;
    for (int c = threadIdx.x; c < width; c += blockDim.x) {
        float s = 0.0f;
        for (int i = 0; i < frame_len; ++i) s += src[(size_t)i * width + c];
        dst[c] = s / (float)frame_len;
    }
}

__global__ void pool_mean_kernel(const float* __restrict__ h, float* __restrict__ out, int t, int width,
                                 const int* __restrict__ lens) {
    const int n = blockIdx.y;
    const int c = blockIdx.x * blockDim.x + threadIdx.x;
    if (c >= width) return;
    const int len = lens ? lens[n] : t;
    const float* src = h + (size_t)n * t * width;
    float s = 0.0f;
    for (int i = 0; i < len; ++i) s += src[(size_t)i * width + c];
    out[(size_t)n * width + c] = s / (float)len;
}

__global__ void zero_pad16_kernel(unsigned short* __restrict__ p, int rows, int ld, int from) {
    const int padw = ld - from;
    const size_t total = (size_t)rows * padw;
    for (size_t i = (size_t)blockIdx.x * blockDim.x + threadIdx.x; i < total; i += (size_t)gridDim.x * blockDim.x) {
        const size_t r = i / padw;
        const int c = (int)(i % padw);
        p[r * ld + from + c] = 0;
    }
}

}

using namespace llark;

extern "C" int llark_prior_embed(const int64_t* z, int n, int t, int width, int bins, const float* x_emb,
                                 const float* pos_emb, const float* x_cond, const float* y_cond, float* h,
                                 llark_stream_t stream) {
    LLARK_REQUIRE(z && x_emb && pos_emb && x_cond && y_cond && h, "prior_embed: null pointer");
    LLARK_REQUIRE(n > 0 && t > 0 && width % 4 == 0, "prior_embed: bad shape n=%d t=%d width=%d", n, t, width);
    const size_t total = (size_t)n * t * (width / 4);
    int grid = (int)((total + 255) / 256);
    if (grid > 256 * 16) grid = 256 * 16;
    prior_embed_kernel<<<grid, 256, 0, (hipStream_t)stream>>>((const long long*)z, (const float4*)x_emb,
                                                                (const float4*)pos_emb, (const float4*)x_cond,
                                                                (const float4*)y_cond, (float4*)h, n, t, width / 4, bins);
    return check_launch("prior_embed");
}

static int layernorm_split_impl(const float* x, int ldx, int rows, int width, const float* gamma, const float* beta, float eps,
                                void* out_hi, void* out_lo, int ldo, int lo8, int ldo8, int sa, llark_stream_t stream) {
    LLARK_REQUIRE(x && gamma && beta && out_hi && out_lo, "layernorm_split: null pointer");
    LLARK_REQUIRE(rows > 0 && width > 0 && width % 4 == 0 && ldx % 4 == 0 && ldo % 4 == 0 && ldo >= width && ldx >= width,
                  "layernorm_split: bad shape rows=%d width=%d ldx=%d ldo=%d", rows, width, ldx, ldo);
    if (lo8) LLARK_REQUIRE(ldo8 % 64 == 0 && ldo8 >= ((width + 63) & ~63) && sa >= 0 && sa <= 40 && ((uintptr_t)out_lo & 3) == 0,
                           "layernorm_split_lo8: ldo8=%d must be a multiple of 64 covering width=%d; sa=%d in [0,40]", ldo8, width, sa);
    const int w4 = width / 4;
    dim3 grid(cdiv(rows, 4));
    hipStream_t s = (hipStream_t)stream;
    if (width % 8 == 0 && ldx % 8 == 0 && ldo % 8 == 0 && ((uintptr_t)out_hi & 15) == 0 && ((uintptr_t)out_lo & (lo8 ? 7 : 15)) == 0 && ((uintptr_t)x & 15) == 0) {
        const int w8 = width / 8;
#define LN8_CASE(NG)                                                                                                                          \
    do {                                                                                                                                      \
        if (lo8) layernorm_split8_kernel<NG, true><<<grid, 256, 0, s>>>(x, ldx, rows, width, gamma, beta, eps, (half_t*)out_hi, (unsigned char*)out_lo, ldo, ldo8, sa);  \
        else layernorm_split8_kernel<NG, false><<<grid, 256, 0, s>>>(x, ldx, rows, width, gamma, beta, eps, (half_t*)out_hi, (unsigned char*)out_lo, ldo, 0, 0);      \
    } while (0)
        if (w8 <= 64) LN8_CASE(1);
        else if (w8 <= 256) LN8_CASE(4);
        else if (w8 <= 640) LN8_CASE(10);
        else if (w8 <= 1024) LN8_CASE(16);
        else { set_error("layernorm_split: width %d too large (max 8192)", width); return LLARK_ERR_UNSUPPORTED; }
#undef LN8_CASE
        return check_launch(lo8 ? "layernorm_split_lo8" : "layernorm_split8");
    }
#define LN_CASE(NV)                                                                                                              \
    do {                                                                                                                         \
        if (lo8) layernorm_split_kernel<NV, true><<<grid, 256, 0, s>>>(x, ldx, rows, width, gamma, beta, eps, (half_t*)out_hi, out_lo, ldo, ldo8, sa); \
        else layernorm_split_kernel<NV, false><<<grid, 256, 0, s>>>(x, ldx, rows, width, gamma, beta, eps, (half_t*)out_hi, out_lo, ldo, 0, 0);   \
    } while (0)
    if (w4 <= 64) LN_CASE(1);
    else if (w4 <= 256) LN_CASE(4);
    else if (w4 <= 1024) LN_CASE(16);
    else if (w4 <= 1216) LN_CASE(19);
    else if (w4 <= 2048) LN_CASE(32);
    else {
        set_error("layernorm_split: width %d too large (max 8192)", width);
        return LLARK_ERR_UNSUPPORTED;
    }
#undef LN_CASE
    return check_launch("layernorm_split");
}

extern "C" int llark_ln_stats_finalize(const float* part, int rows, int nparts, int width, float eps, float* stat, llark_stream_t stream) {
    LLARK_REQUIRE(part && stat && rows > 0 && nparts > 0 && width > 0, "ln_stats_finalize: bad arguments");
    ln_stats_finalize_kernel<<<cdiv(rows, 256), 256, 0, (hipStream_t)stream>>>(part, rows, nparts, width, eps, stat);
    return check_launch("ln_stats_finalize");
}

extern "C" int llark_ln_stats_finalize_p(const float* part, int rows, int nparts, int width, float eps, float* stat, float* pred, llark_stream_t stream) {
    LLARK_REQUIRE(part && stat && pred && rows > 0 && nparts > 0 && width > 0, "ln_stats_finalize_p: bad arguments");
    ln_stats_finalize_p_kernel<<<cdiv(rows, 256), 256, 0, (hipStream_t)stream>>>(part, rows, nparts, width, eps, stat, pred);
    return check_launch("ln_stats_finalize_p");
}

extern "C" int llark_ln_row_pred(const float* x, int ldx, int rows, int width, float eps, float* pred, llark_stream_t stream) {
    LLARK_REQUIRE(x && pred && rows > 0 && width > 0 && width % 4 == 0 && ldx % 4 == 0 && ((uintptr_t)x & 15) == 0,
                  "ln_row_pred: bad arguments (width, ldx multiples of 4, x 16-byte aligned)");
    ln_row_pred_kernel<<<cdiv(rows, 4), 256, 0, (hipStream_t)stream>>>(x, ldx, rows, width, eps, pred);
    return check_launch("ln_row_pred");
}

extern "C" int llark_layernorm_split_f16(const float* x, int ldx, int rows, int width, const float* gamma,
                                         const float* beta, float eps, void* out_hi, void* out_lo, int ldo,
                                         llark_stream_t stream) {
    return layernorm_split_impl(x, ldx, rows, width, gamma, beta, eps, out_hi, out_lo, ldo, 0, 0, 0, stream);
}

extern "C" int llark_layernorm_split_lo8(const float* x, int ldx, int rows, int width, const float* gamma,
                                         const float* beta, float eps, void* out_hi, int ldo, void* out_lo8, int ldo8, int sa,
                                         llark_stream_t stream) {
    return layernorm_split_impl(x, ldx, rows, width, gamma, beta, eps, out_hi, out_lo8, ldo, 1, ldo8, sa, stream);
}

static int prior_attn_impl(const float* qkv, int ldq, int n, int t, int n_state, int heads, int blocks,
                           int pattern, void* out_hi, void* out_lo, int ldo, int lo8, int ldo8, int sa, llark_stream_t stream) {
    LLARK_REQUIRE(qkv && out_hi && out_lo, "prior_attn: null pointer");
    LLARK_REQUIRE(n > 0 && t > 0 && heads > 0 && n_state % heads == 0 && blocks > 0 && t % blocks == 0,
                  "prior_attn: bad shape");
    LLARK_REQUIRE(pattern >= 1 && pattern <= 3, "prior_attn: pattern must be 1 (block), 2 (transpose) or 3 (prev), got %d", pattern);
    const int hd = n_state / heads, bc = t / blocks;
    LLARK_REQUIRE(hd <= 160, "prior_attn: head_dim %d > 160 unsupported", hd);
    LLARK_REQUIRE(bc <= 64, "prior_attn: block_ctx %d > 64 unsupported", bc);
    LLARK_REQUIRE(ldq >= 3 * n_state && ldo >= n_state, "prior_attn: leading dimensions too small");
    AttnParams p;
    p.qkv = qkv; p.ldq = ldq; p.ohi = (half_t*)out_hi; p.olo = (half_t*)out_lo; p.ldo = ldo;
    p.lo8 = lo8; p.ldo8 = ldo8; p.sa = sa;
    if (lo8) LLARK_REQUIRE(ldo8 % 64 == 0 && ldo8 >= ((n_state + 63) & ~63) && sa >= 0 && sa <= 40 && ((uintptr_t)out_lo & 1) == 0,
                           "prior_attn_lo8: ldo8=%d must be a multiple of 64 covering n_state=%d; sa=%d in [0,40]", ldo8, n_state, sa);
    p.T = t; p.n_state = n_state; p.hd = hd; p.heads = heads; p.block_ctx = bc; p.blocks = blocks; p.pattern = pattern;
    p.qc = blocks < 64 ? blocks : 64;
    LLARK_REQUIRE(blocks % p.qc == 0 && blocks <= 128, "prior_attn: blocks=%d must be <=128 and a multiple of %d", blocks, p.qc);
    p.scale2 = (float)(1.0 / sqrt((double)hd));
    {
        double sc = 1.0 / sqrt(sqrt((double)hd));
        p.scale2 = (float)(sc * sc);
    }
    p.hdp = 0;
    p.nk_max = (pattern == 2 && blocks > 64) ? 128 : 64;
    int gx = (pattern == 2) ? bc * (blocks / p.qc) : blocks;
    LLARK_REQUIRE(p.nk_max <= 128, "prior_attn: at most 128 keys per query group (got %d)", p.nk_max);
    LLARK_REQUIRE(hd % 2 == 0 && n_state % 2 == 0 && ldq % 2 == 0 && ldo % 2 == 0,
                  "prior_attn: head_dim, n_state, ldq and ldo must be even (8-byte row loads, 4-byte stores)");
    dim3 grid(gx, heads, n);
#ifndef PRIOR_ATTN_FP32
    {
        const size_t lds16 = 2 * (size_t)a16::PLANE;
        static_assert(2 * a16::PLANE >= 64 * ATT_KP * (int)sizeof(float), "the output stage reuses the planes as a [64][ATT_KP] float tile");
        const int need32 = (hd + 31) / 32;
#define ATT16_LAUNCH(NK)                                                                                                   \
    do {                                                                                                                   \
        static PerDeviceOnce once;                                                                                         \
        if (once.first()) (void)hipFuncSetAttribute((const void*)prior_attn16_kernel<NK>, hipFuncAttributeMaxDynamicSharedMemorySize, (int)lds16); \
        prior_attn16_kernel<NK><<<grid, 256, lds16, (hipStream_t)stream>>>(p);                                             \
    } while (0)
        if (need32 <= 1) ATT16_LAUNCH(1);
        else if (need32 <= 2) ATT16_LAUNCH(2);
        else if (need32 <= 3) ATT16_LAUNCH(3);
        else if (need32 <= 4) ATT16_LAUNCH(4);
        else ATT16_LAUNCH(5);
#undef ATT16_LAUNCH
        return check_launch("prior_attn16");
    }
#endif
    size_t lds = (size_t)64 * ATT_KP * sizeof(float);
    LLARK_REQUIRE(lds <= 160 * 1024, "prior_attn: LDS %zu B exceeds 160 KiB", lds);
    const int need = (hd + 15) / 16;
#define ATT_LAUNCH(NKS)                                                                                              \
    do {                                                                                                             \
        (void)hipFuncSetAttribute((const void*)prior_attn_kernel<NKS>, hipFuncAttributeMaxDynamicSharedMemorySize, (int)lds); \
        prior_attn_kernel<NKS><<<grid, 256, lds, (hipStream_t)stream>>>(p);                                           \
    } while (0)
    if (need <= 2) ATT_LAUNCH(2);
    else if (need <= 4) ATT_LAUNCH(4);
    else if (need <= 8) ATT_LAUNCH(8);
    else ATT_LAUNCH(10);
#undef ATT_LAUNCH
    return check_launch("prior_attn");
}

extern "C" int llark_prior_attn(const float* qkv, int ldq, int n, int t, int n_state, int heads, int blocks,
                                int pattern, void* out_hi, void* out_lo, int ldo, llark_stream_t stream) {
    return prior_attn_impl(qkv, ldq, n, t, n_state, heads, blocks, pattern, out_hi, out_lo, ldo, 0, 0, 0, stream);
}

extern "C" int llark_prior_attn_lo8(const float* qkv, int ldq, int n, int t, int n_state, int heads, int blocks,
                                    int pattern, void* out_hi, int ldo, void* out_lo8, int ldo8, int sa, llark_stream_t stream) {
    return prior_attn_impl(qkv, ldq, n, t, n_state, heads, blocks, pattern, out_hi, out_lo8, ldo, 1, ldo8, sa, stream);
}

extern "C" int llark_pool_window(const float* h, int n, int t, int width, int frame_len, float* out, int frames,
                                 llark_stream_t stream) {
    LLARK_REQUIRE(h && out && n > 0 && frame_len > 0 && frames > 0, "pool_window: bad arguments");
    LLARK_REQUIRE((long)frames * frame_len <= t, "pool_window: %d frames of %d exceed %d rows", frames, frame_len, t);
    dim3 grid(frames, n);
    pool_window_kernel<<<grid, 256, 0, (hipStream_t)stream>>>(h, out, t, width, frame_len, frames);
    return check_launch("pool_window");
}

extern "C" int llark_pool_mean(const float* h, int n, int t, int width, const int* lens, float* out,
                               llark_stream_t stream) {
    LLARK_REQUIRE(h && out && n > 0 && t > 0 && width > 0, "pool_mean: bad arguments");
    dim3 grid(cdiv(width, 256), n);
    pool_mean_kernel<<<grid, 256, 0, (hipStream_t)stream>>>(h, out, t, width, lens);
    return check_launch("pool_mean");
}

extern "C" int llark_zero_pad16(void* plane, int rows, int ld, int from, llark_stream_t stream) {
    LLARK_REQUIRE(plane && rows > 0 && ld >= from && from >= 0, "zero_pad16: bad arguments");
    if (ld == from) return LLARK_OK;
    const size_t total = (size_t)rows * (ld - from);
    int grid = (int)((total + 255) / 256);
    if (grid > 4096) grid = 4096;
    zero_pad16_kernel<<<grid, 256, 0, (hipStream_t)stream>>>((unsigned short*)plane, rows, ld, from);
    return check_launch("zero_pad16");
}
```

llark_amd/jukebox/prior.py:

```python
from __future__ import annotations

import os
from typing import Dict, List, Optional

import numpy as np
import torch

from .. import ops
from .hparams import JukeboxHParams


DEFAULT_PRECISION = "f16x2"

DEFAULT_LN_FOLD = True
DEFAULT_LN_PRED = True
DEFAULT_CPROJ_BDA = False


class Labeller:

    def __init__(self, hps: JukeboxHParams):
        self.hps = hps
        self.sample_length = hps.n_ctx * hps.raw_to_tokens

    def get_label(self, artist, genre, lyrics, total_length, offset):
        del lyrics
        if artist != "unknown" or genre != "unknown":
            raise NotImplementedError("only artist/genre 'unknown' (ids 0) are supported; the v3 id tables are "
                                      "not part of the reference tree")
        y = [total_length, offset, self.sample_length, 0, 0] + [-1] * (self.hps.max_bow_genre_size - 1)
        return dict(y=np.array(y, dtype=np.int64))

    def get_batch_labels(self, metas, device="cpu"):
        ys = [self.get_label(**m)["y"] for m in metas]
        return dict(y=torch.from_numpy(np.stack(ys, axis=0)).to(device).long(), info=None)


class _LayerWeights:
    __slots__ = ("ln0_g", "ln0_b", "ln1_g", "ln1_b", "w_attn", "b_attn", "w_proj", "b_proj", "w_fc", "b_fc", "w_proj2",
                 "b_proj2", "sw_attn", "sw_proj", "sw_fc", "sw_proj2", "w8_attn", "w8_proj", "w8_fc", "w8_proj2",
                 "gw_attn", "bw_attn", "gw_fc", "bw_fc", "wf_proj")


class PriorTransformer:

    def __init__(self, hps: JukeboxHParams, weights: Dict[str, torch.Tensor], device, depth: Optional[int] = None,
                 precision: Optional[str] = None, ln_fold: Optional[bool] = None):
        self.hps = hps
        self.device = torch.device(device)
        self.only_encode = False
        precision = precision or os.environ.get("LLARK_PRIOR_PRECISION", DEFAULT_PRECISION)
        if precision not in ("f16x2", "lo8"):
            raise ValueError(f"prior precision must be 'f16x2' or 'lo8', got {precision!r}")
        self.precision = precision
        if ln_fold is None:
            ln_fold = os.environ.get("LLARK_PRIOR_LN_FOLD", "1" if DEFAULT_LN_FOLD else "0") != "0"
        self.ln_fold = bool(ln_fold) and precision == "f16x2"
        self.ln_pred = self.ln_fold and os.environ.get("LLARK_PRIOR_LN_PRED", "1" if DEFAULT_LN_PRED else "0") != "0"
        self.cproj_bda = self.ln_fold and os.environ.get("LLARK_PRIOR_CPROJ_BDA", "1" if DEFAULT_CPROJ_BDA else "0") != "0"
        self.width = hps.prior_width
        self.depth = hps.prior_depth if depth is None else depth
        dev = self.device

        def f32(name):
            return weights[name].detach().to(device=dev, dtype=torch.float32).contiguous()

        def w16(name):
            w = weights[name].detach().to(device=dev)
            if w.dtype != torch.float16:
                w = w.to(torch.float16)
            wt = ops.pack_weight16(w.contiguous(), transpose=True, dst_dtype=torch.float16, kmult=64 if precision == "lo8" else 32)
            if precision == "lo8" and wt.shape[1] < 128:
                wt = torch.nn.functional.pad(wt, (0, 128 - wt.shape[1])).contiguous()
            return wt

        self.x_emb = f32("prior.x_emb.weight")
        self.pos_emb = f32("prior.pos_emb.pos_emb")
        self.layers: List[_LayerWeights] = []
        for d in range(self.depth):
            p = f"prior.transformer._attn_mods.{d}"
            L = _LayerWeights()
            L.ln0_g, L.ln0_b = f32(f"{p}.ln_0.weight"), f32(f"{p}.ln_0.bias")
            L.ln1_g, L.ln1_b = f32(f"{p}.ln_1.weight"), f32(f"{p}.ln_1.bias")
            L.w_attn, L.b_attn = w16(f"{p}.attn.c_attn.w"), f32(f"{p}.attn.c_attn.b")
            L.w_proj, L.b_proj = w16(f"{p}.attn.c_proj.w"), f32(f"{p}.attn.c_proj.b")
            L.w_fc, L.b_fc = w16(f"{p}.mlp.c_fc.w"), f32(f"{p}.mlp.c_fc.b")
            L.w_proj2, L.b_proj2 = w16(f"{p}.mlp.c_proj.w"), f32(f"{p}.mlp.c_proj.b")
            if precision == "lo8":
                L.sw_attn, L.sw_proj = ops.lo8_weight_exponent(L.w_attn), ops.lo8_weight_exponent(L.w_proj)
                L.sw_fc, L.sw_proj2 = ops.lo8_weight_exponent(L.w_fc), ops.lo8_weight_exponent(L.w_proj2)
                L.w8_attn, L.w8_proj = ops.pack_weight_lo8(L.w_attn, L.sw_attn), ops.pack_weight_lo8(L.w_proj, L.sw_proj)
                L.w8_fc, L.w8_proj2 = ops.pack_weight_lo8(L.w_fc, L.sw_fc), ops.pack_weight_lo8(L.w_proj2, L.sw_proj2)
            if self.ln_fold:
                W = hps.prior_width
                for tag, wt, b, g, be in (("attn", L.w_attn, L.b_attn, L.ln0_g, L.ln0_b), ("fc", L.w_fc, L.b_fc, L.ln1_g, L.ln1_b)):
                    w64 = wt[:, :W].double()
                    setattr(L, "gw_" + tag, (w64 @ g.double()).float().contiguous())
                    setattr(L, "bw_" + tag, (w64 @ be.double() + b.double()).float().contiguous())
                    del w64
            self.layers.append(L)
        self._ws: Dict[str, torch.Tensor] = {}
        self._ws_rows = 0
        self._fold_rows = False

    def _workspace(self, rows: int):
        if self._ws_rows != rows:
            hps, dev = self.hps, self.device
            W, S, Mw = hps.prior_width, hps.n_state, hps.mlp_state
            if self.precision == "lo8":
                Sp, Mp, Wp = (max(128, ops.round_up(v, 64)) for v in (S, Mw, W))
            else:
                Sp, Mp, Wp = ops.round_up(S, 32), ops.round_up(Mw, 32), ops.round_up(W, 32)
            lo_dt = torch.uint8 if self.precision == "lo8" else torch.float16
            ws = {}
            ws["ln_hi"] = torch.zeros((rows, Wp), dtype=torch.float16, device=dev)
            ws["ln_lo"] = torch.zeros((rows, Wp), dtype=lo_dt, device=dev)
            ws["qkv"] = torch.empty((rows, 3 * S), dtype=torch.float32, device=dev)
            ws["att_hi"] = torch.zeros((rows, Sp), dtype=torch.float16, device=dev)
            ws["att_lo"] = torch.zeros((rows, Sp), dtype=lo_dt, device=dev)
            ws["g_hi"] = torch.zeros((rows, Mp), dtype=torch.float16, device=dev)
            ws["g_lo"] = torch.zeros((rows, Mp), dtype=lo_dt, device=dev)
            self._fold_rows = bool(self.ln_fold and all(ops.gemm16_ln_takes(rows, nn, kk) for nn, kk in
                                                        ((3 * S, Wp), (W, Sp), (Mw, Wp), (W, Mp))))
            if self._fold_rows:
                self._ln_parts = 2 * ((W + 255) // 256)
                ws["ln_part"] = torch.empty((rows, max(self._ln_parts, (W + 63) // 64 if self.cproj_bda else 0), 2), dtype=torch.float32, device=dev)
                ws["ln_stat"] = torch.empty((rows, 2), dtype=torch.float32, device=dev)
                ws["ln_pred"] = torch.empty((rows, 2), dtype=torch.float32, device=dev) if self.ln_pred else None
            self._ws, self._ws_rows = ws, rows
        return self._ws

    def layer_forward(self, h2: torch.Tensor, d: int, n: int, taps: Optional[dict] = None, fold_in: bool = False,
                      fold_out: Optional[int] = None) -> None:
        hps, L = self.hps, self.layers[d]
        rows = h2.shape[0]
        ws = self._workspace(rows)
        W, S, Mw = hps.prior_width, hps.n_state, hps.mlp_state
        if self.precision == "lo8":
            return self._layer_forward_lo8(h2, L, d, n, ws, taps)
        if self._fold_rows and taps is None:
            return self._layer_forward_fold(h2, L, d, n, ws, fold_in, fold_out)
        assert not fold_in, "fold_in without the folded path"
        ops.layernorm_split(h2, L.ln0_g, L.ln0_b, 1e-5, ws["ln_hi"], ws["ln_lo"])
        ops.gemm16(ws["ln_hi"], ws["ln_lo"], L.w_attn, L.b_attn, 3 * S, ops.EPI_F32, c=ws["qkv"])
        ops.prior_attn(ws["qkv"], n, hps.n_ctx, S, hps.heads, hps.blocks, [1, 2, 3][d % 3], ws["att_hi"], ws["att_lo"])
        if taps is not None:
            taps["ln0"] = ws["ln_hi"].float() + ws["ln_lo"].float()
            taps["qkv"] = ws["qkv"].clone()
            taps["att"] = (ws["att_hi"].float() + ws["att_lo"].float())[:, :S]
        ops.gemm16(ws["att_hi"], ws["att_lo"], L.w_proj, L.b_proj, W, ops.EPI_RESID, c=h2, resid=h2)
        if taps is not None:
            taps["xa"] = h2.clone()
        ops.layernorm_split(h2, L.ln1_g, L.ln1_b, 1e-5, ws["ln_hi"], ws["ln_lo"])
        ops.gemm16(ws["ln_hi"], ws["ln_lo"], L.w_fc, L.b_fc, Mw, ops.EPI_QGELU_SPLIT, out_hi=ws["g_hi"], out_lo=ws["g_lo"])
        if taps is not None:
            taps["ln1"] = ws["ln_hi"].float() + ws["ln_lo"].float()
            taps["g"] = (ws["g_hi"].float() + ws["g_lo"].float())[:, :Mw]
        ops.gemm16(ws["g_hi"], ws["g_lo"], L.w_proj2, L.b_proj2, W, ops.EPI_RESID, c=h2, resid=h2)

    def _layer_forward_fold(self, h2, L, d: int, n: int, ws, fold_in: bool, fold_out: Optional[int]) -> None:
        hps = self.hps
        W, S, Mw = hps.prior_width, hps.n_state, hps.mlp_state
        rows, part, stat, pred = h2.shape[0], ws["ln_part"], ws["ln_stat"], ws["ln_pred"]
        if pred is not None and not fold_in:
            ops.ln_row_pred(h2, 1e-5, pred)
        if fold_in:
            ops.gemm16_ln(ws["ln_hi"], ws["ln_lo"], L.w_attn, L.bw_attn, 3 * S, ops.EPI_F32, L.gw_attn, ln_stat=stat, c=ws["qkv"])
        else:
            ops.layernorm_split(h2, L.ln0_g, L.ln0_b, 1e-5, ws["ln_hi"], ws["ln_lo"])
            ops.gemm16(ws["ln_hi"], ws["ln_lo"], L.w_attn, L.b_attn, 3 * S, ops.EPI_F32, c=ws["qkv"])
        ops.prior_attn(ws["qkv"], n, hps.n_ctx, S, hps.heads, hps.blocks, [1, 2, 3][d % 3], ws["att_hi"], ws["att_lo"])
        if self.cproj_bda:
            if getattr(L, "wf_proj", None) is None:
                L.wf_proj = ops.pack_weight16_frag(L.w_proj, W)
            np1 = ops.gemm16_lnp_fragw(ws["att_hi"], ws["att_lo"], L.wf_proj, L.b_proj, W, L.w_proj.shape[1], L.ln1_g, part, h2, h2,
                                       ws["ln_hi"], ws["ln_lo"], ln_pred=pred)
        else:
            np1 = self._ln_parts
            ops.gemm16_ln(ws["att_hi"], ws["att_lo"], L.w_proj, L.b_proj, W, ops.EPI_RESID, L.ln1_g, ln_part=part, c=h2, resid=h2,
                          out_hi=ws["ln_hi"], out_lo=ws["ln_lo"], ln_pred=pred)
        ops.ln_stats_finalize(part, rows, np1, W, 1e-5, stat, pred)
        ops.gemm16_ln(ws["ln_hi"], ws["ln_lo"], L.w_fc, L.bw_fc, Mw, ops.EPI_QGELU_SPLIT, L.gw_fc, ln_stat=stat,
                      out_hi=ws["g_hi"], out_lo=ws["g_lo"])
        if fold_out is None:
            ops.gemm16(ws["g_hi"], ws["g_lo"], L.w_proj2, L.b_proj2, W, ops.EPI_RESID, c=h2, resid=h2)
            return
        ops.gemm16_ln(ws["g_hi"], ws["g_lo"], L.w_proj2, L.b_proj2, W, ops.EPI_RESID, self.layers[fold_out].ln0_g, ln_part=part,
                      c=h2, resid=h2, out_hi=ws["ln_hi"], out_lo=ws["ln_lo"], ln_pred=pred)
        ops.ln_stats_finalize(part, rows, self._ln_parts, W, 1e-5, stat, pred)

    def _layer_forward_lo8(self, h2, L, d: int, n: int, ws, taps) -> None:
        hps = self.hps
        W, S, Mw = hps.prior_width, hps.n_state, hps.mlp_state

        def full(hi, lo8, width):
            return hi.float()[:, :width] + ops.lo8_decode(lo8, width)

        ops.layernorm_split_lo8(h2, L.ln0_g, L.ln0_b, 1e-5, ws["ln_hi"], ws["ln_lo"])
        ops.gemm16_lo8(ws["ln_hi"], ws["ln_lo"], L.w_attn, L.sw_attn, L.b_attn, 3 * S, ops.EPI_F32, c=ws["qkv"], w8=L.w8_attn)
        ops.prior_attn(ws["qkv"], n, hps.n_ctx, S, hps.heads, hps.blocks, [1, 2, 3][d % 3], ws["att_hi"], ws["att_lo"])
        if taps is not None:
            taps["ln0"] = full(ws["ln_hi"], ws["ln_lo"], W)
            taps["qkv"] = ws["qkv"].clone()
            taps["att"] = full(ws["att_hi"], ws["att_lo"], S)
        ops.gemm16_lo8(ws["att_hi"], ws["att_lo"], L.w_proj, L.sw_proj, L.b_proj, W, ops.EPI_RESID, c=h2, resid=h2, w8=L.w8_proj)
        if taps is not None:
            taps["xa"] = h2.clone()
        ops.layernorm_split_lo8(h2, L.ln1_g, L.ln1_b, 1e-5, ws["ln_hi"], ws["ln_lo"])
        ops.gemm16_lo8(ws["ln_hi"], ws["ln_lo"], L.w_fc, L.sw_fc, L.b_fc, Mw, ops.EPI_QGELU_SPLIT8, out_hi=ws["g_hi"], out_lo8=ws["g_lo"], w8=L.w8_fc)
        if taps is not None:
            taps["ln1"] = full(ws["ln_hi"], ws["ln_lo"], W)
            taps["g"] = full(ws["g_hi"], ws["g_lo"], Mw)
        ops.gemm16_lo8(ws["g_hi"], ws["g_lo"], L.w_proj2, L.sw_proj2, L.b_proj2, W, ops.EPI_RESID, c=h2, resid=h2, w8=L.w8_proj2)

    def embed(self, x: torch.Tensor, x_cond: torch.Tensor, y_cond: torch.Tensor) -> torch.Tensor:
        n, t = x.shape
        xc = x_cond.reshape(-1, self.width)[:t].contiguous()
        yc = y_cond.reshape(-1)[: self.width].contiguous()
        return ops.prior_embed(x.contiguous(), self.x_emb, self.pos_emb, xc, yc)

    def forward(self, x, x_cond=None, y_cond=None, encoder_kv=None, fp16=False, depth: Optional[int] = None):
        if not self.only_encode:
            raise NotImplementedError("only the only_encode=True path of the prior is implemented (jukebox/main.py:105)")
        if encoder_kv is not None or fp16:
            raise NotImplementedError("encoder_kv / fp16=True are not used by the reference path (jukebox/main.py:108)")
        assert x_cond is not None and y_cond is not None, "top-level prior is conditioned (x_cond=y_pos, y_cond)"
        x = x.to(self.device)
        n, t = x.shape
        assert t == self.hps.n_ctx, f"expected {self.hps.n_ctx} tokens, got {t}"
        h = self.embed(x, x_cond[0:1] if x_cond.dim() == 3 else x_cond, y_cond)
        h2 = h.view(n * t, self.width)
        nd = self.depth if depth is None else depth
        fold = self._workspace(n * t) is not None and self._fold_rows
        for d in range(nd):
            self.layer_forward(h2, d, n, fold_in=fold and d > 0, fold_out=d + 1 if fold and d + 1 < nd else None)
        return h

    __call__ = forward


class TopPrior:

    def __init__(self, hps: JukeboxHParams, weights: Dict[str, torch.Tensor], device="cuda", depth: Optional[int] = None,
                 precision: Optional[str] = None, ln_fold: Optional[bool] = None):
        hps.check()
        self.hps = hps
        self.device = torch.device(device)
        self.raw_to_tokens = hps.raw_to_tokens
        self.n_ctx = hps.n_ctx
        self.labeller = Labeller(hps)
        self.prior = PriorTransformer(hps, weights, device, depth, precision, ln_fold)
        dev = self.device
        self._y_emb = {k.split(".")[1]: v.detach().to(device=dev, dtype=torch.float32).contiguous()
                       for k, v in weights.items() if k.startswith("y_emb.")}
        self._cond_cache = None

    def get_y(self, labels, start, get_indices=False):
        y = labels["y"].clone()
        y[:, 2] = int(self.n_ctx * self.raw_to_tokens)
        y[:, 1:2] = y[:, 1:2] + int(start * self.raw_to_tokens)
        return y

    def _range_bins(self, n_time: int, rng, pos_start: np.ndarray, pos_end=None, clamp=False) -> np.ndarray:
        pos_min, pos_max = np.float32(rng[0]), np.float32(rng[1])
        pos_start = pos_start.astype(np.float32)
        if pos_end is not None:
            pos_end = pos_end.astype(np.float32)
            if clamp:
                pos_end = np.clip(pos_end, pos_min, pos_max)
        if n_time != 1:
            interpolation = (np.arange(0, n_time, dtype=np.float32).reshape(1, n_time) / np.float32(n_time))
            position = pos_start + (pos_end - pos_start) * interpolation
        else:
            position = pos_start
        normalised = (position - pos_min) / (pos_max - pos_min)
        return np.floor(np.float32(self.hps.t_bins) * normalised.astype(np.float32)).astype(np.int64)

    def get_cond(self, z_conds, y):
        assert z_conds is None, "the top-level prior has no upsampler conditioner"
        hps, dev = self.hps, self.device
        yc = y.detach().cpu().numpy().astype(np.int64)
        key = yc.tobytes()
        if self._cond_cache is not None and self._cond_cache[0] == key:
            return self._cond_cache[1]
        n_all = yc.shape[0]
        same = bool((yc == yc[0:1]).all())
        if same:
            yc = yc[0:1]
        total_length, offset, length, artist, genre = yc[:, 0:1], yc[:, 1:2], yc[:, 2:3], yc[:, 3:4], yc[:, 4:]
        E = self._y_emb
        artist_emb = E["artist_emb"][torch.from_numpy(artist).to(dev)]
        mask = torch.from_numpy((genre >= 0).astype(np.float32)).to(dev).unsqueeze(2)
        genre_emb = (E["bow_genre_emb"][torch.from_numpy(np.clip(genre, 0, None)).to(dev)] * mask).sum(dim=1, keepdim=True)
        start_emb = genre_emb + artist_emb
        start, end = offset, offset + length
        tl, st, en = total_length.astype(np.float32), start.astype(np.float32), end.astype(np.float32)
        sr = hps.sr
        r0 = (hps.min_duration * sr, hps.max_duration * sr)
        r1 = (0.0, hps.max_duration * sr)
        r2 = (0.0, 1.0)
        b0 = self._range_bins(1, r0, tl)
        b1 = self._range_bins(hps.n_ctx, r1, st, en)
        b2 = self._range_bins(hps.n_ctx, r2, st / tl, en / tl, clamp=True)
        t = torch.from_numpy
        pos_emb = (E["total_length_emb"][t(b0).to(dev)] + E["absolute_pos_emb"][t(b1).to(dev)]) + E["relative_pos_emb"][t(b2).to(dev)]
        pos_emb, start_emb = pos_emb.contiguous(), start_emb.contiguous()
        if same and n_all > 1:
            pos_emb = pos_emb.expand(n_all, -1, -1)
            start_emb = start_emb.expand(n_all, -1, -1)
        out = (pos_emb, start_emb, None)
        self._cond_cache = (key, out)
        return out
```

llark_amd/ops.py:

```python
from __future__ import annotations

import os
from typing import Optional, Tuple

import torch

from . import _lib
from ._lib import check

F16, BF16, F32SRC = 0, 1, 2
EPI_F32, EPI_RESID, EPI_QGELU_SPLIT, EPI_OUT16, EPI_SWIGLU16, EPI_SPLIT16, EPI_SWIGLU_SPLIT, EPI_QGELU_SPLIT8 = 0, 1, 2, 3, 4, 5, 6, 7
LO8_SA = 12

_DT = {torch.float16: F16, torch.bfloat16: BF16, torch.float32: F32SRC}


_TIMERS = None


def start_kernel_timing() -> None:
    global _TIMERS
    _TIMERS = {}


# ... 156 lines not shown
                                        _dev(b2, "b2", torch.float32), dil, _dev(out, "out", torch.float32), _stream()),
          "resblock")
    return out


def vqvae_weight_exponent(w: torch.Tensor) -> int:
    import math

    amax = float(w.detach().abs().max().float())
    if not (amax > 0.0) or amax != amax:
        return 0
    return max(-40, min(40, 14 - math.ceil(math.log2(amax))))


def vqvae_pack_frag16(w: torch.Tensor, perm1x1: bool = False, exp2: int = 0):
    cout, cin, k = w.shape
    assert cout % 32 == 0 and cin % 16 == 0
    numel = (cout // 32) * (k * cin // 16) * 512
    hi = torch.empty((numel,), dtype=torch.float16, device=w.device)
    lo = torch.empty_like(hi)
    check(_lib.lib().llark_vqvae_pack_frag16(_dev(w, "w", torch.float32), cout, cin, k, int(perm1x1), int(exp2), _dev(hi, "hi"), _dev(lo, "lo"),
                                             _stream()), "vqvae_pack_frag16")
    return hi, lo


def vqvae_stage(x, n: int, cin: int, tin: int, st: dict, out_planes=None, out_f32: Optional[torch.Tensor] = None) -> None:
    import ctypes

    if cin == 1:
        audio, in_hi, in_lo = _dev(x, "audio", torch.float32), None, None
        assert x.numel() >= n * tin
    else:
        audio, in_hi, in_lo = None, _dev(x[0], "in_hi", torch.float16), _dev(x[1], "in_lo", torch.float16)
        assert x[0].numel() >= n * tin * cin and x[1].numel() >= n * tin * cin
    c = 64 if st["wo_hi"] is not None else 32
    need = n * (tin // 2) * c
    if out_planes is not None:
        assert out_planes[0].numel() >= need and out_planes[1].numel() >= need
    if out_f32 is not None:
        assert out_f32.numel() >= need
    dil = (ctypes.c_int * len(st["dil"]))(*st["dil"])
    wexp = (ctypes.c_int * len(st["wexp"]))(*st["wexp"])
    assert len(st["wexp"]) == 2 + 2 * len(st["dil"])
    opt = lambda t, name, dt: _dev(t, name, dt) if t is not None else None
    check(_lib.lib().llark_vqvae_stage_f16x2(
        audio, in_hi, in_lo, n, cin, tin, opt(st["w0f"], "w0f", torch.float32), opt(st["w0_hi"], "w0_hi", torch.float16),
        opt(st["w0_lo"], "w0_lo", torch.float16), _dev(st["b0"], "b0", torch.float32), _dev(st["wr_hi"], "wr_hi", torch.float16),
        _dev(st["wr_lo"], "wr_lo", torch.float16), _dev(st["br"], "br", torch.float32), len(st["dil"]),
        ctypes.cast(dil, ctypes.c_void_p), opt(st["wo_hi"], "wo_hi", torch.float16), opt(st["wo_lo"], "wo_lo", torch.float16),
        opt(st["bo"], "bo", torch.float32), ctypes.cast(wexp, ctypes.c_void_p), out_planes[0].data_ptr() if out_planes is not None else None,
        out_planes[1].data_ptr() if out_planes is not None else None, out_f32.data_ptr() if out_f32 is not None else None, _stream()),
        "vqvae_stage")


def codebook_norms(k: torch.Tensor) -> torch.Tensor:
    bins, emb = k.shape
    kk = torch.empty((bins,), dtype=torch.float32, device=k.device)
    check(_lib.lib().llark_codebook_norms_f32(_dev(k, "k", torch.float32), bins, emb, _dev(kk, "kk"), _stream()),
          "codebook_norms")
    return kk


def codebook_argmin(x: torch.Tensor, k: torch.Tensor, kk: torch.Tensor, want_dist: bool = False):
    n, emb, t = x.shape
    bins = k.shape[0]
    codes = torch.empty((n, t), dtype=torch.int64, device=x.device)
    dist = torch.empty((n, t), dtype=torch.float32, device=x.device) if want_dist else None
    check(_lib.lib().llark_codebook_argmin(_dev(x, "x", torch.float32), n, emb, t, _dev(k, "k", torch.float32),
                                           _dev(kk, "kk", torch.float32), bins, _dev(codes, "codes"),
                                           dist.data_ptr() if dist is not None else None, _stream()), "codebook_argmin")
    return (codes, dist) if want_dist else codes


def codebook_argmin_tie(x: torch.Tensor, k: torch.Tensor, kk: torch.Tensor, tie_a: float, tie_b: float, flag_count: torch.Tensor,
                        flag_list: torch.Tensor, codes: Optional[torch.Tensor] = None) -> torch.Tensor:
    n, emb, t = x.shape
    if codes is None:
        codes = torch.empty((n, t), dtype=torch.int64, device=x.device)
    check(_lib.lib().llark_codebook_argmin_tie(_dev(x, "x", torch.float32), n, emb, t, _dev(k, "k", torch.float32), _dev(kk, "kk", torch.float32),
                                               k.shape[0], _dev(codes, "codes", torch.int64), float(tie_a), float(tie_b),
                                               _dev(flag_count, "flag_count", torch.int32), _dev(flag_list, "flag_list", torch.int32),
                                               flag_list.numel(), _stream()), "codebook_argmin_tie")
    return codes


def vqvae_fix_near_ties(plan, audio: torch.Tensor, raw_to_tokens: int, flag_list: torch.Tensor, count: int, halo_tokens: int, win_tokens: int,
                        win: torch.Tensor, col: torch.Tensor, buf0: torch.Tensor, buf1: torch.Tensor, k: torch.Tensor, kk: torch.Tensor,
                        codes: torch.Tensor) -> None:
    n, t = audio.shape
    assert win.numel() >= count * win_tokens * raw_to_tokens and col.numel() >= count and buf0.numel() == buf1.numel()
    check(_lib.lib().llark_vqvae_fix_near_ties(plan, _dev(audio, "audio", torch.float32), n, t, raw_to_tokens, _dev(flag_list, "flag_list", torch.int32),
                                               int(count), int(halo_tokens), int(win_tokens), _dev(win, "win", torch.float32),
                                               _dev(col, "col", torch.int32), _dev(buf0, "buf0", torch.float32), _dev(buf1, "buf1", torch.float32),
                                               buf0.numel(), _dev(k, "k", torch.float32), _dev(kk, "kk", torch.float32), k.shape[0],
                                               _dev(codes, "codes", torch.int64), _stream()), "vqvae_fix_near_ties")


def prior_embed(z, x_emb, pos_emb, x_cond, y_cond, out: Optional[torch.Tensor] = None) -> torch.Tensor:
    n, t = z.shape
    bins, width = x_emb.shape
    assert pos_emb.shape == (t, width) and x_cond.numel() == t * width and y_cond.numel() == width
    if out is None:
        out = torch.empty((n, t, width), dtype=torch.float32, device=z.device)
    check(_lib.lib().llark_prior_embed(_dev(z, "z", torch.int64), n, t, width, bins, _dev(x_emb, "x_emb", torch.float32),
                                       _dev(pos_emb, "pos_emb", torch.float32), _dev(x_cond, "x_cond", torch.float32),
                                       _dev(y_cond, "y_cond", torch.float32), _dev(out, "h", torch.float32), _stream()),
          "prior_embed")
    return out


def layernorm_split(x: torch.Tensor, gamma, beta, eps: float, out_hi: torch.Tensor, out_lo: torch.Tensor) -> None:
    rows, width = x.shape
    assert out_hi.shape == out_lo.shape and out_hi.shape[0] == rows and out_hi.shape[1] >= width
    check(_lib.lib().llark_layernorm_split_f16(_dev(x, "x", torch.float32), x.stride(0), rows, width,
                                               _dev(gamma, "gamma", torch.float32), _dev(beta, "beta", torch.float32),
                                               float(eps), _dev(out_hi, "out_hi", torch.float16),
                                               _dev(out_lo, "out_lo", torch.float16), out_hi.stride(0), _stream()),
          "layernorm_split")


def layernorm_split_lo8(x: torch.Tensor, gamma, beta, eps: float, out_hi: torch.Tensor, out_lo8: torch.Tensor, sa: int = LO8_SA) -> None:
    rows, width = x.shape
    assert out_hi.shape[0] == rows and out_lo8.shape[0] == rows and out_hi.shape[1] >= width and out_lo8.dtype == torch.uint8
    check(_lib.lib().llark_layernorm_split_lo8(_dev(x, "x", torch.float32), x.stride(0), rows, width,
                                               _dev(gamma, "gamma", torch.float32), _dev(beta, "beta", torch.float32),
                                               float(eps), _dev(out_hi, "out_hi", torch.float16), out_hi.stride(0),
                                               _dev(out_lo8, "out_lo8", torch.uint8), out_lo8.stride(0), int(sa), _stream()),
          "layernorm_split_lo8")


def lo8_decode(lo8: torch.Tensor, width: int, sa: int = LO8_SA) -> torch.Tensor:
    rows, ld = lo8.shape
    k = torch.arange(ld, device=lo8.device)
    r = k & 63
    pos = (k & ~63) + (((r >> 3) & 1) << 5) + ((r >> 4) << 3) + (r & 7)
    b = lo8[:, pos][:, :width].to(torch.int32)
    e, mnt = (b >> 3) & 15, (b & 7).float()
    mag = torch.where(e == 0, mnt * 2.0 ** -9, (1.0 + mnt * 0.125) * torch.exp2(e.float() - 7.0))
    return torch.where((b & 128) != 0, -mag, mag) * (2.0 ** -sa)


def prior_attn(qkv: torch.Tensor, n: int, t: int, n_state: int, heads: int, blocks: int, pattern: int,
               out_hi: torch.Tensor, out_lo: torch.Tensor, lo8_sa: Optional[int] = None) -> None:
    assert qkv.shape[0] == n * t and qkv.shape[1] >= 3 * n_state
    if out_lo.dtype == torch.uint8:
        check(_lib.lib().llark_prior_attn_lo8(_dev(qkv, "qkv", torch.float32), qkv.stride(0), n, t, n_state, heads, blocks,
                                              pattern, _dev(out_hi, "out_hi", torch.float16), out_hi.stride(0),
                                              _dev(out_lo, "out_lo8", torch.uint8), out_lo.stride(0),
                                              LO8_SA if lo8_sa is None else int(lo8_sa), _stream()), "prior_attn_lo8")
        return
    check(_lib.lib().llark_prior_attn(_dev(qkv, "qkv", torch.float32), qkv.stride(0), n, t, n_state, heads, blocks,
                                      pattern, _dev(out_hi, "out_hi", torch.float16), _dev(out_lo, "out_lo", torch.float16),
                                      out_hi.stride(0), _stream()), "prior_attn")


def pool_window(h: torch.Tensor, frame_len: int, frames: int) -> torch.Tensor:
    n, t, width = h.shape
    out = torch.empty((n, frames, width), dtype=torch.float32, device=h.device)
    check(_lib.lib().llark_pool_window(_dev(h, "h", torch.float32), n, t, width, frame_len, _dev(out, "out"), frames,
                                       _stream()), "pool_window")
    return out


def pool_mean(h: torch.Tensor, lens: Optional[torch.Tensor] = None) -> torch.Tensor:
    n, t, width = h.shape
    out = torch.empty((n, width), dtype=torch.float32, device=h.device)
    lp = _dev(lens, "lens", torch.int32) if lens is not None else None
    check(_lib.lib().llark_pool_mean(_dev(h, "h", torch.float32), n, t, width, lp, _dev(out, "out"), _stream()),
          "pool_mean")
    return out


def pack_weight16(w: torch.Tensor, transpose: bool, dst_dtype: torch.dtype, kmult: int = 32) -> torch.Tensor:
    if transpose:
        k, n = w.shape
    else:
        n, k = w.shape
    kp = round_up(k, kmult)
    wt = torch.empty((n, kp), dtype=dst_dtype, device=w.device)
    check(_lib.lib().llark_pack_weight16(_dev(w, "w"), _DT[w.dtype], int(transpose), k, n, _dev(wt, "wt"), _DT[dst_dtype],
                                         kp, _stream()), "pack_weight16")
    return wt


def split16(x: torch.Tensor, dtype: torch.dtype, want_lo: bool = True, kmult: int = 32):
    rows, width = x.shape
    ldo = round_up(width, kmult)
    hi = torch.empty((rows, ldo), dtype=dtype, device=x.device)
    lo = torch.empty((rows, ldo), dtype=dtype, device=x.device) if want_lo else None
    check(_lib.lib().llark_split16(_DT[dtype], _dev(x, "x", torch.float32), x.stride(0), rows, width, _dev(hi, "hi"),
                                   lo.data_ptr() if lo is not None else None, ldo, _stream()), "split16")
    return hi, lo


GEMV_DMA = os.environ.get("LLARK_GEMV_DMA", "1") == "1"
GEMV_DMA_MIN_BYTES = 64 * 1000 * 1000
FRAG_MIN_ROWS = int(os.environ.get("LLARK_FRAG_MIN_ROWS", "129"))


def attach_frag(wt: torch.Tensor, n: int) -> None:
    if wt.shape[1] % 64 or wt.stride(1) != 1 or os.environ.get("LLARK_FRAG", "1") == "0":
        return
    wt._llark_frag = (pack_weight16_frag(wt, n), n, wt.shape[1])


def detach_frag(wt: torch.Tensor) -> None:
    if hasattr(wt, "_llark_frag"):
        del wt._llark_frag


def refresh_frag(wt: torch.Tensor) -> None:
    fr = getattr(wt, "_llark_frag", None)
    if fr is not None:
        pack_weight16_frag(wt, fr[1], out=fr[0])


def _gemv_dma_takes(split: bool, m: int, kp: int) -> bool:
    if m < 1 or m > 4 or kp % 8 or kp > 12288:
        return False
    if kp <= 4096 and m <= 2:
        return True
    mm = m if m <= 2 else 4
    return mm * (2 if split else 1) * ((kp + 4095) // 4096) * 8192 <= 48 * 1024


def gemm16(a_hi: torch.Tensor, a_lo: Optional[torch.Tensor], wt: torch.Tensor, bias: Optional[torch.Tensor], n: int,
           epilogue: int, c: Optional[torch.Tensor] = None, resid: Optional[torch.Tensor] = None,
           out_hi: Optional[torch.Tensor] = None, out_lo: Optional[torch.Tensor] = None, m: Optional[int] = None,
           variant: int = -1) -> None:
    dtype = a_hi.dtype
    assert dtype in (torch.float16, torch.bfloat16) and wt.dtype == dtype
    m = a_hi.shape[0] if m is None else m
    kp = wt.shape[1]
    assert a_hi.shape[1] >= kp and wt.shape[0] >= n, f"gemm16: A has {a_hi.shape[1]} cols, wt {tuple(wt.shape)}, n={n}"
    name = ("gemm_split_" if a_lo is not None else "gemm_") + ("f16" if dtype == torch.float16 else "bf16") + ("_skinny" if m <= 16 else "")
    if epilogue == EPI_SWIGLU_SPLIT and out_lo is None:
        raise ValueError("gemm16: EPI_SWIGLU_SPLIT needs out_lo")
    if (variant < 0 and GEMV_DMA and dtype == torch.bfloat16 and n * kp * 2 >= GEMV_DMA_MIN_BYTES and _gemv_dma_takes(a_lo is not None, m, kp)
            and epilogue in (EPI_F32, EPI_RESID, EPI_SWIGLU16, EPI_SWIGLU_SPLIT) and a_hi.stride(0) % 8 == 0 and wt.stride(0) % 8 == 0):
        with _timed(name, 2.0 * m * n * kp):
            check(_lib.lib().llark_gemv16_dma(
                int(a_lo is not None), epilogue, _dev(a_hi, "a_hi"), _dev(a_lo, "a_lo", dtype) if a_lo is not None else None, a_hi.stride(0),
                _dev(wt, "wt"), wt.stride(0), _dev(bias, "bias", torch.float32) if bias is not None else None, m, n, kp,
                _dev(c, "c", torch.float32) if c is not None else None, c.stride(0) if c is not None else 0,
                _dev(resid, "resid", torch.float32) if resid is not None else None, resid.stride(0) if resid is not None else 0,
                _dev(out_hi, "out_hi", dtype) if out_hi is not None else None, _dev(out_lo, "out_lo", dtype) if out_lo is not None else None,
                out_hi.stride(0) if out_hi is not None else 0, _stream()), "gemv16_dma")
        return
    if variant < 0 and m >= FRAG_MIN_ROWS:
        fr = getattr(wt, "_llark_frag", None)
        if fr is not None and fr[1] == n and fr[2] == kp:
            return gemm16_fragw(a_hi, a_lo, fr[0], bias, n, kp, epilogue, c=c, resid=resid, out_hi=out_hi, out_lo=out_lo, m=m)
    with _timed(name, 2.0 * m * n * kp):
      check(_lib.lib().llark_gemm16_ws(
        variant, _DT[dtype], int(a_lo is not None), epilogue, _dev(a_hi, "a_hi"), _dev(a_lo, "a_lo", dtype) if a_lo is not None else None,
        a_hi.stride(0), _dev(wt, "wt"), wt.stride(0), _dev(bias, "bias", torch.float32) if bias is not None else None,
        m, n, kp, _dev(c, "c", torch.float32) if c is not None else None, c.stride(0) if c is not None else 0,
        _dev(resid, "resid", torch.float32) if resid is not None else None, resid.stride(0) if resid is not None else 0,
        _dev(out_hi, "out_hi", dtype) if out_hi is not None else None,
        _dev(out_lo, "out_lo", dtype) if out_lo is not None else None,
        out_hi.stride(0) if out_hi is not None else 0, workspace(), _stream()), "gemm16")


def gemm16_ln_takes(m: int, n: int, kp: int) -> bool:
    return bool(_lib.lib().llark_gemm16_ln_takes(int(m), int(n), int(kp)))


def gemm16_ln(a_hi: torch.Tensor, a_lo: torch.Tensor, wt: torch.Tensor, bias: Optional[torch.Tensor], n: int, epilogue: int,
              ln_vec: torch.Tensor, ln_stat: Optional[torch.Tensor] = None, ln_part: Optional[torch.Tensor] = None,
              c: Optional[torch.Tensor] = None, resid: Optional[torch.Tensor] = None, out_hi: Optional[torch.Tensor] = None,
              out_lo: Optional[torch.Tensor] = None, m: Optional[int] = None, ln_pred: Optional[torch.Tensor] = None) -> None:
    dtype = a_hi.dtype
    assert dtype in (torch.float16, torch.bfloat16) and wt.dtype == dtype and a_lo is not None
    m = a_hi.shape[0] if m is None else m
    kp = wt.shape[1]
    assert a_hi.shape[1] >= kp and wt.shape[0] >= n and ln_vec.numel() >= n
    if ln_part is not None:
        assert ln_part.numel() >= m * 2 * ((n + 255) // 256) * 2, "gemm16_ln: ln_part is [m][2 * ceil(n / 256)][2]"
    if ln_stat is not None:
        assert ln_stat.numel() >= 2 * m
    if ln_pred is not None:
        assert ln_part is not None and ln_pred.numel() >= 2 * m and ln_pred.is_contiguous()
    name = "gemm_split_" + ("f16" if dtype == torch.float16 else "bf16")
    with _timed(name, 2.0 * m * n * kp):
        check(_lib.lib().llark_gemm16_ln_p(
            _DT[dtype], epilogue, _dev(a_hi, "a_hi"), _dev(a_lo, "a_lo", dtype), a_hi.stride(0), _dev(wt, "wt"), wt.stride(0),
            _dev(bias, "bias", torch.float32) if bias is not None else None, m, n, kp,
            _dev(c, "c", torch.float32) if c is not None else None, c.stride(0) if c is not None else 0,
            _dev(resid, "resid", torch.float32) if resid is not None else None, resid.stride(0) if resid is not None else 0,
            _dev(out_hi, "out_hi", dtype) if out_hi is not None else None, _dev(out_lo, "out_lo", dtype) if out_lo is not None else None,
            out_hi.stride(0) if out_hi is not None else 0,
            _dev(ln_stat, "ln_stat", torch.float32) if ln_stat is not None else None, _dev(ln_vec, "ln_vec", torch.float32),
            _dev(ln_part, "ln_part", torch.float32) if ln_part is not None else None,
            _dev(ln_pred, "ln_pred", torch.float32) if ln_pred is not None else None, workspace(), _stream()), "gemm16_ln")


def gemm16_lnp_fragw(a_hi: torch.Tensor, a_lo: torch.Tensor, wfrag: torch.Tensor, bias: Optional[torch.Tensor], n: int, kp: int,
                     ln_vec: torch.Tensor, ln_part: torch.Tensor, c: torch.Tensor, resid: torch.Tensor, out_hi: torch.Tensor,
                     out_lo: torch.Tensor, m: Optional[int] = None, ln_pred: Optional[torch.Tensor] = None) -> int:
    dtype = a_hi.dtype
    assert dtype in (torch.float16, torch.bfloat16) and wfrag.dtype == dtype and a_hi.shape[1] >= kp
    assert wfrag.numel() == round_up(n, 32) * kp and ln_vec.numel() >= n
    m = a_hi.shape[0] if m is None else m
    nparts = (n + 63) // 64
    assert ln_part.numel() >= m * nparts * 2, "gemm16_lnp_fragw: ln_part is [m][ceil(n / 64)][2]"
    if ln_pred is not None:
# ... 795 lines not shown
```

Baseline: 12.63 clips/s.

## Emit QKV as padded fp16 hi/lo planes and add plane-based prior attention kernel

The QKV projection GEMM in the folded prior path now writes fp16 hi/lo split planes, padded per head to multiples of 8, instead of an fp32 qkv buffer. A new attention kernel reads these planes with buffer-load-to-LDS and MFMA, and runs several work items per block with prefetch of the next item. This is meant to cut the fp32 qkv write and read traffic and the in-kernel fp32 to fp16 split. In exchange it adds per-layer permuted weight copies, a new kernel with shape restrictions, and a fallback path.

```diff
diff --git a/include/llark_hip.h b/include/llark_hip.h
--- a/include/llark_hip.h
+++ b/include/llark_hip.h
@@ -75,6 +75,8 @@
                               float eps, void* out_hi, void* out_lo, int ldo, llark_stream_t stream);
 int llark_prior_attn(const float* qkv, int ldq, int n, int t, int n_state, int heads, int blocks, int pattern,
                      void* out_hi, void* out_lo, int ldo, llark_stream_t stream);
+int llark_prior_attn_planes(const void* qkv_hi, const void* qkv_lo, int ldq, int n, int t, int n_state, int heads, int blocks,
+                            int pattern, void* out_hi, void* out_lo, int ldo, int run, llark_stream_t stream);
 int llark_layernorm_split_lo8(const float* x, int ldx, int rows, int width, const float* gamma, const float* beta,
                               float eps, void* out_hi, int ldo, void* out_lo8, int ldo8, int sa, llark_stream_t stream);
 int llark_prior_attn_lo8(const float* qkv, int ldq, int n, int t, int n_state, int heads, int blocks, int pattern,
diff --git a/llark_amd/_lib.py b/llark_amd/_lib.py
--- a/llark_amd/_lib.py
+++ b/llark_amd/_lib.py
@@ -45,6 +45,7 @@
     "llark_prior_embed": [_P, c_int, c_int, c_int, c_int, _P, _P, _P, _P, _P, _P],
     "llark_layernorm_split_f16": [_P, c_int, c_int, c_int, _P, _P, c_float, _P, _P, c_int, _P],
     "llark_prior_attn": [_P, c_int, c_int, c_int, c_int, c_int, c_int, c_int, _P, _P, c_int, _P],
+    "llark_prior_attn_planes": [_P, _P, c_int, c_int, c_int, c_int, c_int, c_int, c_int, _P, _P, c_int, c_int, _P],
     "llark_pool_window": [_P, c_int, c_int, c_int, c_int, _P, c_int, _P],
     "llark_pool_mean": [_P, c_int, c_int, c_int, _P, _P, _P],
     "llark_zero_pad16": [_P, c_int, c_int, c_int, _P],
diff --git a/llark_amd/csrc/gemm.hip b/llark_amd/csrc/gemm.hip
--- a/llark_amd/csrc/gemm.hip
+++ b/llark_amd/csrc/gemm.hip
@@ -823,7 +823,7 @@
     LLARK_REQUIRE((ln_stat != nullptr) != (ln_part != nullptr), "gemm16_ln: exactly one of ln_stat (consumer) / ln_part (producer) must be given");
     LLARK_REQUIRE(lda % 8 == 0 && ldw % 8 == 0 && lda >= kp && ldw >= kp, "gemm16_ln: lda/ldw must be >= kp and multiples of 8");
     if (ln_part) LLARK_REQUIRE(epilogue == EPI_RESID && c && resid && out_hi && out_lo && ldc >= n && ldr >= n && ldo >= n, "gemm16_ln: the producer role is LLARK_EPI_RESID with c, resid and the operand planes");
-    else LLARK_REQUIRE((epilogue == EPI_F32 && c && ldc >= n) || (epilogue == EPI_QGELU_SPLIT && out_hi && out_lo && ldo >= n), "gemm16_ln: the consumer role is LLARK_EPI_F32 or LLARK_EPI_QGELU_SPLIT");
+    else LLARK_REQUIRE((epilogue == EPI_F32 && c && ldc >= n) || ((epilogue == EPI_QGELU_SPLIT || epilogue == EPI_SPLIT16) && out_hi && out_lo && ldo >= n), "gemm16_ln: the consumer role is LLARK_EPI_F32, LLARK_EPI_QGELU_SPLIT or LLARK_EPI_SPLIT16");
     if (!gemm256x_takes(m, n, kp) || ws->cus % 8) {
         set_error("gemm16_ln: m=%d n=%d kp=%d is not a shape the 256x256 tile takes", m, n, kp);
         return LLARK_ERR_UNSUPPORTED;
diff --git a/llark_amd/csrc/gemm256x.hip b/llark_amd/csrc/gemm256x.hip
--- a/llark_amd/csrc/gemm256x.hip
+++ b/llark_amd/csrc/gemm256x.hip
@@ -549,6 +549,7 @@
         if (!p.ln_vec || p.ln_part) return -1000;
         if (epi == EPI_F32) return launch256x<T, EPI_F32, 1>(p, s, cus);
         if (epi == EPI_QGELU_SPLIT) return launch256x<T, EPI_QGELU_SPLIT, 1>(p, s, cus);
+        if (epi == EPI_SPLIT16 && p.act == 0 && p.Ohi2 == nullptr) return launch256x<T, EPI_SPLIT16, 1>(p, s, cus);
         return -1000;
     }
     if (p.ln_part) {
diff --git a/llark_amd/csrc/prior.hip b/llark_amd/csrc/prior.hip
--- a/llark_amd/csrc/prior.hip
+++ b/llark_amd/csrc/prior.hip
@@ -764,6 +764,316 @@
     }
 }
 
+#ifndef PRIOR_ATTN_PLANES_RUN
+#define PRIOR_ATTN_PLANES_RUN 2
+#endif
+struct AttnPlanesParams {
+    const half_t* qhi;
+    const half_t* qlo;
+    int ldq;
+    unsigned nbytes;
+    half_t* ohi;
+    half_t* olo;
+    int ldo;
+    int T, n_state, hd, hs, heads, block_ctx, blocks, pattern, qc;
+    float scale2;
+    int run;
+    int nitems;
+};
+
+struct AttnItem {
+    int nq, q0, qs, nkeys, k0, ks, coff, ntile;
+    bool causal, zero_out;
+};
+__device__ __forceinline__ AttnItem attn_item(const AttnPlanesParams& p, int x) {
+    AttnItem it;
+    it.causal = true;
+    it.zero_out = false;
+    if (p.pattern == 1) {
+        it.nq = p.block_ctx; it.q0 = x * p.block_ctx; it.qs = 1;
+        it.nkeys = p.block_ctx; it.k0 = it.q0; it.ks = 1; it.coff = 0;
+    } else if (p.pattern == 2) {
+        const int chunks = p.blocks / p.qc;
+        int off, ch;
+        if (PRIOR_ATTN_P2_XCD && (p.block_ctx & 7) == 0) {
+            off = (x & 7) + 8 * (x / (8 * chunks));
+            ch = chunks - 1 - (x >> 3) % chunks;
+        } else {
+            off = x / chunks;
+            ch = x % chunks;
+        }
+        it.nq = p.qc; it.q0 = ch * p.qc * p.block_ctx + off; it.qs = p.block_ctx;
+        it.nkeys = (ch + 1) * p.qc; it.k0 = off; it.ks = p.block_ctx; it.coff = ch * p.qc;
+    } else {
+        it.nq = p.block_ctx; it.q0 = x * p.block_ctx; it.qs = 1;
+        it.nkeys = p.block_ctx; it.k0 = (x - 1) * p.block_ctx; it.ks = 1; it.coff = 0;
+        it.causal = false;
+        it.zero_out = (x == 0);
+    }
+    it.ntile = (it.nkeys + 63) >> 6;
+    return it;
+}
+
+template <int NK32>
+__global__ __launch_bounds__(256) __attribute__((amdgpu_waves_per_eu(2, 2))) void prior_attn_planes_kernel(const AttnPlanesParams p) {
+    extern __shared__ __attribute__((aligned(16))) float sm[];
+    char* tile = (char*)sm;
+    const int tid = threadIdx.x;
+    const int lane = tid & 63, g = lane >> 4, c = lane & 15;
+    const int wv = __builtin_amdgcn_readfirstlane(tid >> 6);
+    const int head = blockIdx.y;
+    const int clip = blockIdx.z;
+    const int hd = p.hd;
+    const int nch = p.hs >> 3;
+    constexpr int NDT = 2 * NK32;
+    typedef _Float16 half2_t __attribute__((ext_vector_type(2)));
+    typedef _Float16 half4_t __attribute__((ext_vector_type(4)));
+    typedef half4_t __attribute__((aligned(4))) half4u_t;
+
+    const bool p2x = p.pattern == 2 && PRIOR_ATTN_P2_XCD && (p.block_ctx & 7) == 0;
+    const int nslot = p2x ? p.nitems >> 3 : p.nitems;
+    const int slot0 = (p2x ? (int)(blockIdx.x >> 3) : (int)blockIdx.x) * p.run;
+    const int xlow = p2x ? (int)(blockIdx.x & 7) : 0, xmul = p2x ? 8 : 1;
+    int nrun = nslot - slot0 < p.run ? nslot - slot0 : p.run;
+    if (nrun <= 0) return;
+    const size_t rowbase = (size_t)clip * p.T;
+    const int ocol = head * hd;
+    const int npad2 = head == p.heads - 1 ? (p.ldo - p.n_state) >> 1 : 0;
+
+    const unsigned RSRC_FLAGS = 0x00020000u;
+    const __amdgpu_buffer_rsrc_t rH = __builtin_amdgcn_make_buffer_rsrc((void*)p.qhi, 0, (int)p.nbytes, RSRC_FLAGS);
+    const __amdgpu_buffer_rsrc_t rL = __builtin_amdgcn_make_buffer_rsrc((void*)p.qlo, 0, (int)p.nbytes, RSRC_FLAGS);
+
+    auto zero_pad_rows = [&](const AttnItem& it) __attribute__((always_inline)) {
+        for (int idx = lane; idx < 16 * npad2; idx += 64) {
+            const int rr = idx / npad2, pr = idx - rr * npad2;
+            const int i = wv * 16 + rr;
+            if (i >= it.nq) break;
+            const size_t o = (rowbase + it.q0 + (size_t)i * it.qs) * p.ldo + p.n_state + 2 * pr;
+            *(half2_t*)(p.ohi + o) = half2_t{(half_t)0.0f, (half_t)0.0f};
+            *(half2_t*)(p.olo + o) = half2_t{(half_t)0.0f, (half_t)0.0f};
+        }
+    };
+
+    int jx = 0;
+    AttnItem cur = attn_item(p, xlow + xmul * slot0);
+    if (cur.zero_out) {
+        for (int i = tid; i < cur.nq * hd; i += 256) {
+            const int r = i / hd, d = i - r * hd;
+            const size_t o = (rowbase + cur.q0 + (size_t)r * cur.qs) * p.ldo + ocol + d;
+            p.ohi[o] = (half_t)0.0f;
+            p.olo[o] = (half_t)0.0f;
+        }
+        zero_pad_rows(cur);
+        if (++jx >= nrun) return;
+        cur = attn_item(p, xlow + xmul * (slot0 + jx));
+    }
+
+    auto issue_half = [&](const AttnItem& it, int s) __attribute__((always_inline)) {
+        const bool isv = s >= 2 * it.ntile;
+        const int r = isv ? s - 2 * it.ntile : s;
+        const int st = r & 1;
+        const unsigned colb = (unsigned)(((isv ? 2 : 1) * p.heads + head) * p.hs) * 2u;
+        const unsigned tokb = (unsigned)(rowbase + it.k0) * (unsigned)(p.ldq * 2) + colb;
+#pragma unroll
+        for (int i = 0; i < 4; ++i) {
+            const int rh = 2 * (wv * 4 + i);
+            const int trow = 32 * st + rh + (lane >> 5);
+            const int key = 32 * r + rh + (lane >> 5);
+            const int chunk = (lane & 31) ^ a16::swz(trow);
+            const bool ok = chunk < nch && key < it.nkeys;
+            const unsigned vo = (tokb + (unsigned)(key * it.ks) * (unsigned)(p.ldq * 2) + (unsigned)(chunk << 4)) | (ok ? 0u : 0x80000000u);
+            const int dst = (32 * st + rh) * a16::PITCH;
+            __builtin_amdgcn_raw_ptr_buffer_load_lds(rH, (__attribute__((address_space(3))) void*)(tile + dst), 16, vo, 0, 0, 0);
+            __builtin_amdgcn_raw_ptr_buffer_load_lds(rL, (__attribute__((address_space(3))) void*)(tile + a16::PLANE + dst), 16, vo, 0, 0, 0);
+        }
+    };
+    half8_t qh[NK32], ql[NK32];
+    auto load_q = [&](const AttnItem& it) __attribute__((always_inline)) {
+        int qr = wv * 16 + c;
+        qr = qr < it.nq ? qr : it.nq - 1;
+        const unsigned o = ((unsigned)(rowbase + it.q0) + (unsigned)(qr * it.qs)) * (unsigned)(p.ldq * 2) + (unsigned)(head * p.hs * 2);
+#pragma unroll
+        for (int s = 0; s < NK32; ++s) {
+            const int chunk = 4 * s + g;
+            const unsigned vo = (o + (unsigned)(chunk << 4)) | (chunk < nch ? 0u : 0x80000000u);
+            qh[s] = __builtin_bit_cast(half8_t, __builtin_amdgcn_raw_buffer_load_b128(rH, vo, 0, 0));
+            ql[s] = __builtin_bit_cast(half8_t, __builtin_amdgcn_raw_buffer_load_b128(rL, vo, 0, 0));
+        }
+    };
+
+    const unsigned lds0 = (unsigned)(uintptr_t)(__attribute__((address_space(3))) char*)tile;
+    auto tr_issue = [&](a16::v4s_t(&f)[4], int row0, int col0) __attribute__((always_inline)) {
+        const int col = col0 + 4 * (c & 3);
+        const int ra = row0 + 8 * g + (c >> 2), rb = ra + 4;
+        const unsigned oa = lds0 + ra * a16::PITCH + ((((col >> 3) ^ a16::swz(ra)) << 4) | ((col & 7) << 1));
+        const unsigned ob = lds0 + rb * a16::PITCH + ((((col >> 3) ^ a16::swz(rb)) << 4) | ((col & 7) << 1));
+        asm volatile("ds_read_b64_tr_b16 %0, %1" : "=v"(f[0]) : "v"(oa));
+        asm volatile("ds_read_b64_tr_b16 %0, %1" : "=v"(f[1]) : "v"(ob));
+        asm volatile("ds_read_b64_tr_b16 %0, %1" : "=v"(f[2]) : "v"(oa + a16::PLANE));
+        asm volatile("ds_read_b64_tr_b16 %0, %1" : "=v"(f[3]) : "v"(ob + a16::PLANE));
+    };
+
+    issue_half(cur, 0);
+    load_q(cur);
+    const int krow = 8 * (c >> 2) + (c & 3);
+    const int kswz = a16::swz(krow);
+
+    for (;;) {
+        const bool has_next = jx + 1 < nrun;
+        const AttnItem nxt = attn_item(p, xlow + xmul * (slot0 + (has_next ? jx + 1 : jx)));
+        const int ntile = cur.ntile, nhalf = 4 * cur.ntile;
+        const int nkeys = cur.nkeys;
+        auto phase_top = [&](int s) __attribute__((always_inline)) {
+            asm volatile("s_waitcnt vmcnt(0) lgkmcnt(0)" ::: "memory");
+            __builtin_amdgcn_s_barrier();
+            asm volatile("" ::: "memory");
+            if (s + 1 < nhalf) issue_half(cur, s + 1);
+            else if (has_next) issue_half(nxt, 0);
+        };
+
+        f32x4_t sc[2][4];
+#pragma unroll
+        for (int kt = 0; kt < 2; ++kt) {
+            if (kt >= ntile) break;
+#pragma unroll
+            for (int h = 0; h < 2; ++h) {
+                phase_top(2 * kt + h);
+                f32x4_t acc[2];
+#pragma unroll
+                for (int u = 0; u < 2; ++u) acc[u] = f32x4_t{0.f, 0.f, 0.f, 0.f};
+#pragma unroll
+                for (int s = 0; s < NK32; ++s) {
+                    half8_t kh[2], kl[2];
+#pragma unroll
+                    for (int u = 0; u < 2; ++u) {
+                        const int o = (krow + 32 * h + 4 * u) * a16::PITCH + (((4 * s + g) ^ kswz) << 4);
+                        kh[u] = *(const half8_t*)(tile + o);
+                        kl[u] = *(const half8_t*)(tile + a16::PLANE + o);
+                    }
+#pragma unroll
+                    for (int u = 0; u < 2; ++u) acc[u] = a16::mfma(kh[u], qh[s], acc[u]);
+#pragma unroll
+                    for (int u = 0; u < 2; ++u) acc[u] = a16::mfma(kh[u], ql[s], acc[u]);
+#pragma unroll
+                    for (int u = 0; u < 2; ++u) acc[u] = a16::mfma(kl[u], qh[s], acc[u]);
+                }
+                const int i = wv * 16 + c;
+#pragma unroll
+                for (int u = 0; u < 2; ++u)
+#pragma unroll
+                    for (int r = 0; r < 4; ++r) {
+                        const int j = kt * 64 + 32 * h + 8 * g + 4 * u + r;
+                        const bool ok = (j < nkeys) && (!cur.causal || (j <= i + cur.coff));
+                        sc[kt][2 * h + u][r] = ok ? acc[u][r] * p.scale2 : -INFINITY;
+                    }
+            }
+        }
+        if (has_next) load_q(nxt);
+
+        {
+            float mx = -INFINITY;
+#pragma unroll
+            for (int kt = 0; kt < 2; ++kt) {
+                if (kt >= ntile) break;
+#pragma unroll
+                for (int t = 0; t < 4; ++t)
+                    mx = fmaxf(fmaxf(fmaxf(sc[kt][t][0], sc[kt][t][1]), fmaxf(sc[kt][t][2], sc[kt][t][3])), mx);
+            }
+            mx = fmaxf(mx, __shfl_xor(mx, 16));
+            mx = fmaxf(mx, __shfl_xor(mx, 32));
+            float sum = 0.0f;
+#pragma unroll
+            for (int kt = 0; kt < 2; ++kt) {
+                if (kt >= ntile) break;
+#pragma unroll
+                for (int t = 0; t < 4; ++t)
+#pragma unroll
+                    for (int r = 0; r < 4; ++r) {
+                        const float ex = mx > -INFINITY ? expf(sc[kt][t][r] - mx) : 0.0f;
+                        sc[kt][t][r] = ex;
+                        sum += ex;
+                    }
+            }
+            sum += __shfl_xor(sum, 16);
+            sum += __shfl_xor(sum, 32);
+            const float inv = sum > 0.0f ? 1.0f / sum : 0.0f;
+#pragma unroll
+            for (int kt = 0; kt < 2; ++kt) {
+                if (kt >= ntile) break;
+#pragma unroll
+                for (int t = 0; t < 4; ++t) sc[kt][t] *= inv;
+            }
+        }
+
+        f32x4_t o[NDT];
+#pragma unroll
+        for (int dt = 0; dt < NDT; ++dt) o[dt] = f32x4_t{0.f, 0.f, 0.f, 0.f};
+#pragma unroll
+        for (int kt = 0; kt < 2; ++kt) {
+            if (kt >= ntile) break;
+#pragma unroll
+            for (int u = 0; u < 2; ++u) {
+                phase_top(2 * ntile + 2 * kt + u);
+                half8_t ph, pl;
+#pragma unroll
+                for (int e = 0; e < 8; ++e) {
+                    const float pv = sc[kt][2 * u + (e >> 2)][e & 3];
+                    const half_t h = (half_t)pv;
+                    ph[e] = h;
+                    pl[e] = (half_t)(pv - (float)h);
+                }
+                a16::v4s_t fr[2][4];
+                tr_issue(fr[0], 32 * u, 0);
+#pragma unroll
+                for (int dt = 0; dt < NDT; ++dt) {
+                    a16::v4s_t(&f)[4] = fr[dt & 1];
+                    if (dt + 1 < NDT) {
+                        tr_issue(fr[(dt + 1) & 1], 32 * u, 16 * (dt + 1));
+                        asm volatile("s_waitcnt lgkmcnt(4)" : "+v"(f[0]), "+v"(f[1]), "+v"(f[2]), "+v"(f[3]));
+                    } else {
+                        asm volatile("s_waitcnt lgkmcnt(0)" : "+v"(f[0]), "+v"(f[1]), "+v"(f[2]), "+v"(f[3]));
+                    }
+                    const a16::v8s_t vh8 = {f[0][0], f[0][1], f[0][2], f[0][3], f[1][0], f[1][1], f[1][2], f[1][3]};
+                    const a16::v8s_t vl8 = {f[2][0], f[2][1], f[2][2], f[2][3], f[3][0], f[3][1], f[3][2], f[3][3]};
+                    const half8_t vh = __builtin_bit_cast(half8_t, vh8), vl = __builtin_bit_cast(half8_t, vl8);
+                    o[dt] = a16::mfma(vh, ph, o[dt]);
+                    o[dt] = a16::mfma(vh, pl, o[dt]);
+                    o[dt] = a16::mfma(vl, ph, o[dt]);
+                }
+            }
+        }
+
+        {
+            const int i = wv * 16 + c;
+            if (i < cur.nq) {
+                const size_t ob = (rowbase + cur.q0 + (size_t)i * cur.qs) * p.ldo + ocol;
+#pragma unroll
+                for (int dt = 0; dt < NDT; ++dt) {
+                    const int d0 = 16 * dt + 4 * g;
+                    half4_t h, l;
+#pragma unroll
+                    for (int r = 0; r < 4; ++r) {
+                        h[r] = (half_t)o[dt][r];
+                        l[r] = (half_t)(o[dt][r] - (float)h[r]);
+                    }
+                    if (d0 + 3 < hd) {
+                        *(half4u_t*)(p.ohi + ob + d0) = h;
+                        *(half4u_t*)(p.olo + ob + d0) = l;
+                    } else if (d0 + 1 < hd) {
+                        *(half2_t*)(p.ohi + ob + d0) = half2_t{h[0], h[1]};
+                        *(half2_t*)(p.olo + ob + d0) = half2_t{l[0], l[1]};
+                    }
+                }
+            }
+            zero_pad_rows(cur);
+        }
+        if (!has_next) break;
+        ++jx;
+        cur = nxt;
+    }
+}
+
 __global__ void pool_window_kernel(const float* __restrict__ h, float* __restrict__ out, int t, int width,
                                    int frame_len, int frames) {
     const int f = blockIdx.x, n = blockIdx.y;
@@ -966,6 +1276,50 @@
     return prior_attn_impl(qkv, ldq, n, t, n_state, heads, blocks, pattern, out_hi, out_lo8, ldo, 1, ldo8, sa, stream);
 }
 
+extern "C" int llark_prior_attn_planes(const void* qkv_hi, const void* qkv_lo, int ldq, int n, int t, int n_state, int heads, int blocks,
+                                       int pattern, void* out_hi, void* out_lo, int ldo, int run, llark_stream_t stream) {
+    LLARK_REQUIRE(qkv_hi && qkv_lo && out_hi && out_lo, "prior_attn_planes: null pointer");
+    LLARK_REQUIRE(n > 0 && t > 0 && heads > 0 && n_state % heads == 0 && blocks > 0 && t % blocks == 0, "prior_attn_planes: bad shape");
+    LLARK_REQUIRE(pattern >= 1 && pattern <= 3, "prior_attn_planes: pattern must be 1 (block), 2 (transpose) or 3 (prev), got %d", pattern);
+    const int hd = n_state / heads, bc = t / blocks, hs = (hd + 7) & ~7;
+    LLARK_REQUIRE(hd <= 160 && hd % 2 == 0, "prior_attn_planes: head_dim %d must be even and <= 160", hd);
+    LLARK_REQUIRE(bc <= 64, "prior_attn_planes: block_ctx %d > 64 unsupported", bc);
+    LLARK_REQUIRE(ldq >= 3 * heads * hs && ldq % 8 == 0 && (((uintptr_t)qkv_hi | (uintptr_t)qkv_lo) & 15) == 0,
+                  "prior_attn_planes: planes must be 16-byte aligned with ldq a multiple of 8 and >= 3 * heads * %d", hs);
+    LLARK_REQUIRE(ldo >= n_state && ldo % 2 == 0 && (((uintptr_t)out_hi | (uintptr_t)out_lo) & 3) == 0, "prior_attn_planes: ldo must be even and >= n_state");
+    LLARK_REQUIRE((long long)n * t * ldq * 2 < (1ll << 31), "prior_attn_planes: a plane must be smaller than 2 GiB (32-bit buffer offsets)");
+    AttnPlanesParams p;
+    p.qhi = (const half_t*)qkv_hi; p.qlo = (const half_t*)qkv_lo; p.ldq = ldq; p.nbytes = (unsigned)((long long)n * t * ldq * 2);
+    p.ohi = (half_t*)out_hi; p.olo = (half_t*)out_lo; p.ldo = ldo;
+    p.T = t; p.n_state = n_state; p.hd = hd; p.hs = hs; p.heads = heads; p.block_ctx = bc; p.blocks = blocks; p.pattern = pattern;
+    p.qc = blocks < 64 ? blocks : 64;
+    LLARK_REQUIRE(blocks % p.qc == 0 && blocks <= 128, "prior_attn_planes: blocks=%d must be <=128 and a multiple of %d", blocks, p.qc);
+    {
+        double sc = 1.0 / sqrt(sqrt((double)hd));
+        p.scale2 = (float)(sc * sc);
+    }
+    p.run = run > 0 ? run : PRIOR_ATTN_PLANES_RUN;
+    p.nitems = (pattern == 2) ? bc * (blocks / p.qc) : blocks;
+    const bool p2x = pattern == 2 && PRIOR_ATTN_P2_XCD && (bc & 7) == 0;
+    const int gx = p2x ? 8 * ((p.nitems / 8 + p.run - 1) / p.run) : (p.nitems + p.run - 1) / p.run;
+    dim3 grid(gx, heads, n);
+    const size_t lds = 2 * (size_t)a16::PLANE;
+    const int need32 = (hs + 31) / 32;
+#define ATTP_LAUNCH(NK)                                                                                                          \
+    do {                                                                                                                         \
+        static PerDeviceOnce once;                                                                                               \
+        if (once.first()) (void)hipFuncSetAttribute((const void*)prior_attn_planes_kernel<NK>, hipFuncAttributeMaxDynamicSharedMemorySize, (int)lds); \
+        prior_attn_planes_kernel<NK><<<grid, 256, lds, (hipStream_t)stream>>>(p);                                                \
+    } while (0)
+    if (need32 <= 1) ATTP_LAUNCH(1);
+    else if (need32 <= 2) ATTP_LAUNCH(2);
+    else if (need32 <= 3) ATTP_LAUNCH(3);
+    else if (need32 <= 4) ATTP_LAUNCH(4);
+    else ATTP_LAUNCH(5);
+#undef ATTP_LAUNCH
+    return check_launch("prior_attn_planes");
+}
+
 extern "C" int llark_pool_window(const float* h, int n, int t, int width, int frame_len, float* out, int frames,
                                  llark_stream_t stream) {
     LLARK_REQUIRE(h && out && n > 0 && frame_len > 0 && frames > 0, "pool_window: bad arguments");
diff --git a/llark_amd/jukebox/prior.py b/llark_amd/jukebox/prior.py
--- a/llark_amd/jukebox/prior.py
+++ b/llark_amd/jukebox/prior.py
@@ -39,7 +39,7 @@
 class _LayerWeights:
     __slots__ = ("ln0_g", "ln0_b", "ln1_g", "ln1_b", "w_attn", "b_attn", "w_proj", "b_proj", "w_fc", "b_fc", "w_proj2",
                  "b_proj2", "sw_attn", "sw_proj", "sw_fc", "sw_proj2", "w8_attn", "w8_proj", "w8_fc", "w8_proj2",
-                 "gw_attn", "bw_attn", "gw_fc", "bw_fc", "wf_proj")
+                 "gw_attn", "bw_attn", "gw_fc", "bw_fc", "wf_proj", "wp_attn", "bp_attn", "gwp_attn", "bwp_attn")
 
 
 class PriorTransformer:
@@ -91,17 +91,44 @@
                 L.sw_fc, L.sw_proj2 = ops.lo8_weight_exponent(L.w_fc), ops.lo8_weight_exponent(L.w_proj2)
                 L.w8_attn, L.w8_proj = ops.pack_weight_lo8(L.w_attn, L.sw_attn), ops.pack_weight_lo8(L.w_proj, L.sw_proj)
                 L.w8_fc, L.w8_proj2 = ops.pack_weight_lo8(L.w_fc, L.sw_fc), ops.pack_weight_lo8(L.w_proj2, L.sw_proj2)
-            if self.ln_fold:
-                W = hps.prior_width
-                for tag, wt, b, g, be in (("attn", L.w_attn, L.b_attn, L.ln0_g, L.ln0_b), ("fc", L.w_fc, L.b_fc, L.ln1_g, L.ln1_b)):
-                    w64 = wt[:, :W].double()
-                    setattr(L, "gw_" + tag, (w64 @ g.double()).float().contiguous())
-                    setattr(L, "bw_" + tag, (w64 @ be.double() + b.double()).float().contiguous())
-                    del w64
             self.layers.append(L)
+        H, hd = hps.heads, hps.n_state // hps.heads
+        hs = ops.round_up(hd, 8)
+        self._attn_np = 3 * H * hs
+        col = torch.arange(3 * hps.n_state, device=dev)
+        self._attn_cols = (col // hd) * hs + col % hd
+        if self.ln_fold:
+            self._derive_fold()
         self._ws: Dict[str, torch.Tensor] = {}
         self._ws_rows = 0
         self._fold_rows = False
+        self._planes_rows = False
+
+    def _derive_fold(self) -> None:
+        W = self.hps.prior_width
+        for L in self.layers:
+            for tag, wt, b, g, be in (("attn", L.w_attn, L.b_attn, L.ln0_g, L.ln0_b), ("fc", L.w_fc, L.b_fc, L.ln1_g, L.ln1_b)):
+                w64 = wt[:, :W].double()
+                for name, val in (("gw_" + tag, (w64 @ g.double()).float()), ("bw_" + tag, (w64 @ be.double() + b.double()).float())):
+                    if getattr(L, name, None) is None:
+                        setattr(L, name, val.contiguous())
+                    else:
+                        getattr(L, name).copy_(val)
+                del w64
+            if getattr(L, "wp_attn", None) is None:
+                L.wp_attn = torch.zeros((self._attn_np, L.w_attn.shape[1]), dtype=L.w_attn.dtype, device=self.device)
+                L.bp_attn, L.gwp_attn, L.bwp_attn = (torch.zeros(self._attn_np, dtype=torch.float32, device=self.device) for _ in range(3))
+            L.wp_attn[self._attn_cols] = L.w_attn[: self._attn_cols.numel()]
+            L.bp_attn[self._attn_cols] = L.b_attn
+            L.gwp_attn[self._attn_cols] = L.gw_attn
+            L.bwp_attn[self._attn_cols] = L.bw_attn
+
+    def weights_changed_in_place(self) -> None:
+        if self.ln_fold:
+            self._derive_fold()
+        for L in self.layers:
+            if getattr(L, "wf_proj", None) is not None:
+                L.wf_proj = None
 
     def _workspace(self, rows: int):
         if self._ws_rows != rows:
@@ -115,13 +142,18 @@
             ws = {}
             ws["ln_hi"] = torch.zeros((rows, Wp), dtype=torch.float16, device=dev)
             ws["ln_lo"] = torch.zeros((rows, Wp), dtype=lo_dt, device=dev)
-            ws["qkv"] = torch.empty((rows, 3 * S), dtype=torch.float32, device=dev)
             ws["att_hi"] = torch.zeros((rows, Sp), dtype=torch.float16, device=dev)
             ws["att_lo"] = torch.zeros((rows, Sp), dtype=lo_dt, device=dev)
             ws["g_hi"] = torch.zeros((rows, Mp), dtype=torch.float16, device=dev)
             ws["g_lo"] = torch.zeros((rows, Mp), dtype=lo_dt, device=dev)
             self._fold_rows = bool(self.ln_fold and all(ops.gemm16_ln_takes(rows, nn, kk) for nn, kk in
                                                         ((3 * S, Wp), (W, Sp), (Mw, Wp), (W, Mp))))
+            hd = S // hps.heads
+            self._planes_rows = bool(self._fold_rows and ops.gemm16_ln_takes(rows, self._attn_np, Wp) and hd % 2 == 0 and hd <= 160
+                                     and hps.n_ctx // hps.blocks <= 64 and rows * self._attn_np * 2 < 2 ** 31)
+            if self._planes_rows:
+                ws["qkv_hi"] = torch.empty((rows, self._attn_np), dtype=torch.float16, device=dev)
+                ws["qkv_lo"] = torch.empty((rows, self._attn_np), dtype=torch.float16, device=dev)
             if self._fold_rows:
                 self._ln_parts = 2 * ((W + 255) // 256)
                 ws["ln_part"] = torch.empty((rows, max(self._ln_parts, (W + 63) // 64 if self.cproj_bda else 0), 2), dtype=torch.float32, device=dev)
@@ -129,6 +161,11 @@
                 ws["ln_pred"] = torch.empty((rows, 2), dtype=torch.float32, device=dev) if self.ln_pred else None
             self._ws, self._ws_rows = ws, rows
         return self._ws
+
+    def _qkv32(self, ws, rows: int) -> torch.Tensor:
+        if "qkv" not in ws:
+            ws["qkv"] = torch.empty((rows, 3 * self.hps.n_state), dtype=torch.float32, device=self.device)
+        return ws["qkv"]
 
     def layer_forward(self, h2: torch.Tensor, d: int, n: int, taps: Optional[dict] = None, fold_in: bool = False,
                       fold_out: Optional[int] = None) -> None:
@@ -141,6 +178,7 @@
         if self._fold_rows and taps is None:
             return self._layer_forward_fold(h2, L, d, n, ws, fold_in, fold_out)
         assert not fold_in, "fold_in without the folded path"
+        self._qkv32(ws, rows)
         ops.layernorm_split(h2, L.ln0_g, L.ln0_b, 1e-5, ws["ln_hi"], ws["ln_lo"])
         ops.gemm16(ws["ln_hi"], ws["ln_lo"], L.w_attn, L.b_attn, 3 * S, ops.EPI_F32, c=ws["qkv"])
         ops.prior_attn(ws["qkv"], n, hps.n_ctx, S, hps.heads, hps.blocks, [1, 2, 3][d % 3], ws["att_hi"], ws["att_lo"])
@@ -164,12 +202,23 @@
         rows, part, stat, pred = h2.shape[0], ws["ln_part"], ws["ln_stat"], ws["ln_pred"]
         if pred is not None and not fold_in:
             ops.ln_row_pred(h2, 1e-5, pred)
-        if fold_in:
-            ops.gemm16_ln(ws["ln_hi"], ws["ln_lo"], L.w_attn, L.bw_attn, 3 * S, ops.EPI_F32, L.gw_attn, ln_stat=stat, c=ws["qkv"])
+        pat = [1, 2, 3][d % 3]
+        if self._planes_rows:
+            Np, qh, ql = self._attn_np, ws["qkv_hi"], ws["qkv_lo"]
+            if fold_in:
+                ops.gemm16_ln(ws["ln_hi"], ws["ln_lo"], L.wp_attn, L.bwp_attn, Np, ops.EPI_SPLIT16, L.gwp_attn, ln_stat=stat, out_hi=qh, out_lo=ql)
+            else:
+                ops.layernorm_split(h2, L.ln0_g, L.ln0_b, 1e-5, ws["ln_hi"], ws["ln_lo"])
+                ops.gemm16(ws["ln_hi"], ws["ln_lo"], L.wp_attn, L.bp_attn, Np, ops.EPI_SPLIT16, out_hi=qh, out_lo=ql)
+            ops.prior_attn_planes(qh, ql, n, hps.n_ctx, S, hps.heads, hps.blocks, pat, ws["att_hi"], ws["att_lo"])
         else:
-            ops.layernorm_split(h2, L.ln0_g, L.ln0_b, 1e-5, ws["ln_hi"], ws["ln_lo"])
-            ops.gemm16(ws["ln_hi"], ws["ln_lo"], L.w_attn, L.b_attn, 3 * S, ops.EPI_F32, c=ws["qkv"])
-        ops.prior_attn(ws["qkv"], n, hps.n_ctx, S, hps.heads, hps.blocks, [1, 2, 3][d % 3], ws["att_hi"], ws["att_lo"])
+            qkv = self._qkv32(ws, rows)
+            if fold_in:
+                ops.gemm16_ln(ws["ln_hi"], ws["ln_lo"], L.w_attn, L.bw_attn, 3 * S, ops.EPI_F32, L.gw_attn, ln_stat=stat, c=qkv)
+            else:
+                ops.layernorm_split(h2, L.ln0_g, L.ln0_b, 1e-5, ws["ln_hi"], ws["ln_lo"])
+                ops.gemm16(ws["ln_hi"], ws["ln_lo"], L.w_attn, L.b_attn, 3 * S, ops.EPI_F32, c=qkv)
+            ops.prior_attn(qkv, n, hps.n_ctx, S, hps.heads, hps.blocks, pat, ws["att_hi"], ws["att_lo"])
         if self.cproj_bda:
             if getattr(L, "wf_proj", None) is None:
                 L.wf_proj = ops.pack_weight16_frag(L.w_proj, W)
@@ -196,6 +245,7 @@
         def full(hi, lo8, width):
             return hi.float()[:, :width] + ops.lo8_decode(lo8, width)
 
+        self._qkv32(ws, h2.shape[0])
         ops.layernorm_split_lo8(h2, L.ln0_g, L.ln0_b, 1e-5, ws["ln_hi"], ws["ln_lo"])
         ops.gemm16_lo8(ws["ln_hi"], ws["ln_lo"], L.w_attn, L.sw_attn, L.b_attn, 3 * S, ops.EPI_F32, c=ws["qkv"], w8=L.w8_attn)
         ops.prior_attn(ws["qkv"], n, hps.n_ctx, S, hps.heads, hps.blocks, [1, 2, 3][d % 3], ws["att_hi"], ws["att_lo"])
diff --git a/llark_amd/ops.py b/llark_amd/ops.py
--- a/llark_amd/ops.py
+++ b/llark_amd/ops.py
@@ -332,6 +332,17 @@
     check(_lib.lib().llark_prior_attn(_dev(qkv, "qkv", torch.float32), qkv.stride(0), n, t, n_state, heads, blocks,
                                       pattern, _dev(out_hi, "out_hi", torch.float16), _dev(out_lo, "out_lo", torch.float16),
                                       out_hi.stride(0), _stream()), "prior_attn")
+
+
+def prior_attn_planes(qkv_hi: torch.Tensor, qkv_lo: torch.Tensor, n: int, t: int, n_state: int, heads: int, blocks: int, pattern: int,
+                      out_hi: torch.Tensor, out_lo: torch.Tensor, run: int = 0) -> None:
+    hs = round_up(n_state // heads, 8)
+    assert qkv_hi.shape == qkv_lo.shape and qkv_hi.stride(0) == qkv_lo.stride(0)
+    assert qkv_hi.shape[0] == n * t and qkv_hi.shape[1] >= 3 * heads * hs
+    assert out_hi.shape == out_lo.shape and out_hi.stride(0) == out_lo.stride(0) and out_hi.shape[1] == out_hi.stride(0)
+    check(_lib.lib().llark_prior_attn_planes(_dev(qkv_hi, "qkv_hi", torch.float16), _dev(qkv_lo, "qkv_lo", torch.float16), qkv_hi.stride(0),
+                                             n, t, n_state, heads, blocks, pattern, _dev(out_hi, "out_hi", torch.float16),
+                                             _dev(out_lo, "out_lo", torch.float16), out_hi.stride(0), int(run), _stream()), "prior_attn_planes")
 
 
 def pool_window(h: torch.Tensor, frame_len: int, frames: int) -> torch.Tensor:
```

Result: no change. 12.68 clips/s, median of 6 (+0.4%).
